# pain7576/ddpg-trucktrailer

Measured on AMD Instinct MI355X. Metric: env-steps/s, higher is better.
Workload: dtype f64

## Files before the change

### ddpg-trucktrailer_amd/_lib.py

```python
import ctypes as C
import os

HERE = os.path.dirname(os.path.abspath(__file__))
LIB_PATH = os.environ.get("TT_LIB_PATH") or os.path.join(HERE, "libttenv.so")

OBS_DIM = 23
MAX_EPISODE_STEPS = 4095
TT_OK, TT_EINVAL, TT_ENOMEM, TT_EHIP, TT_ENODEV = 0, -1, -2, -3, -4
F_JACKKNIFE, F_OUT_OF_MAP, F_MAX_STEPS, F_GOAL_REACHED, F_GOAL_PASSED, F_EXCESSIVE_BACK, F_SUCCESS = (1 << i for i in range(7))
VIOLATIONS = ("none", "jackknife", "jackknife_warning", "major_boundary", "minor_boundary", "past_the_goal",
              "max_step", "excessive_backward")
INFO_ROWS = ("total_reward", "progress_reward", "heading_reward", "orientation_reward", "staged_success",
             "safety_penalty", "exploration_bonus", "final_success_bonus", "backward_penalty", "smoothness_penalty",
             "cumulative_backward", "movement_budget")
NINFO = len(INFO_ROWS)
LOG_COUNTS = ("episodes", "successes", "jackknife", "out_of_map", "max_steps", "goal_reached", "goal_passed",
              "excessive_back", "success_flag")
LOG_DETAIL = 1
LOG_COMPONENTS = INFO_ROWS[1:10]


class TTParams(C.Structure):
    _fields_ = [(n, C.c_double) for n in ("L1", "L2", "hitch_offset", "v1x", "dt", "map_min_x", "map_max_x", "map_min_y",
                                          "map_max_y", "max_steer", "position_threshold", "orientation_threshold",
                                          "step_length")] + \
               [("extra_steps", C.c_int32), ("fixed_max_steps", C.c_int32), ("term_mask", C.c_uint32),
                ("variant", C.c_int32), ("stateless_reward", C.c_int32), ("reserved_", C.c_int32),
                ("goal", C.c_double * 3), ("reset_lo", C.c_double * 3),
                ("reset_hi", C.c_double * 3)]


class TTInfo(C.Structure):
    _fields_ = [("comp", C.c_void_p), ("violation", C.c_void_p), ("flags", C.c_void_p)]


class TTMlpWeights(C.Structure):
    _fields_ = [(n, C.c_void_p) for n in ("w1", "b1", "g1", "be1", "w2", "b2", "g2", "be2", "w3", "b3", "wa", "ba")] + \
               [("in_dim", C.c_int32), ("fc1_dims", C.c_int32), ("fc2_dims", C.c_int32), ("capped_grids", C.c_int32),
                ("split_ws", C.c_void_p), ("ws_packed", C.c_int32), ("max_workgroups", C.c_int32), ("split_ws_alt", C.c_void_p), ("fc2_img", C.c_void_p)]


class TTFc2Images(C.Structure):
    _fields_ = [("net", C.c_void_p), ("target", C.c_void_p)]


class TTMlpSaved(C.Structure):
    _fields_ = [(n, C.c_void_p) for n in ("xh1", "h1", "xh2", "h2", "rstd1", "rstd2")]


class TTFwdJob(C.Structure):
    _fields_ = [("critic", C.c_int32), ("reserved_", C.c_int32), ("obs", C.c_void_p), ("action", C.c_void_p),
                ("w", C.POINTER(TTMlpWeights)), ("out", C.c_void_p), ("saved", C.POINTER(TTMlpSaved)),
                ("dq_da", C.c_void_p), ("z_state", C.c_void_p)]


class TTTdInput(C.Structure):
    _fields_ = [("z_state", C.c_void_p), ("mu_target", C.c_void_p), ("target_critic", C.POINTER(TTMlpWeights)),
                ("reward", C.c_void_p), ("done", C.c_void_p), ("gamma", C.c_float), ("reserved_", C.c_float),
                ("y_out", C.c_void_p), ("q_out", C.c_void_p), ("step_dev", C.c_void_p), ("window_dev", C.c_void_p),
                ("bias_corr_out", C.c_void_p), ("adam_beta1", C.c_float), ("adam_beta2", C.c_float)]


class TTSideBuffer(C.Structure):
    _fields_ = [("obs", C.c_void_p), ("act", C.c_void_p), ("rew", C.c_void_p), ("obs2", C.c_void_p), ("done", C.c_void_p),
                ("count", C.c_int32), ("reserved_", C.c_int32)]


class TTRingView(C.Structure):
    _fields_ = [("cursor", C.c_void_p), ("obs", C.c_void_p), ("act", C.c_void_p), ("rew", C.c_void_p), ("done", C.c_void_p),
                ("n_envs", C.c_int32), ("slots", C.c_int32)]


class TTRingCursor(C.Structure):
    _fields_ = [("k_dev", C.c_void_p), ("slots", C.c_int32), ("reserved_", C.c_int32), ("cursor", C.c_void_p)]


class TTSampleArgs(C.Structure):
    _fields_ = [("batch", C.c_int32), ("n_envs", C.c_int32), ("slots", C.c_int32), ("reserve", C.c_int32), ("k_dev", C.c_void_p),
                ("obs", C.c_void_p), ("act", C.c_void_p), ("rew", C.c_void_p), ("done", C.c_void_p), ("seed", C.c_uint64),
                ("side", C.POINTER(TTSideBuffer)), ("s_out", C.c_void_p), ("a_out", C.c_void_p), ("r_out", C.c_void_p),
                ("s2_out", C.c_void_p), ("d_out", C.c_void_p), ("idx_out", C.c_void_p), ("lag", C.c_int32),
                ("draws", C.c_int32), ("seed_stride", C.c_uint64), ("step_progress", C.c_void_p)]


class TTImageJob(C.Structure):
    _fields_ = [("actor", C.POINTER(TTMlpWeights)), ("cursor", C.POINTER(TTRingCursor))]


class TTMlpBwdWs(C.Structure):
    _fields_ = [(n, C.c_void_p) for n in ("dpre", "dz", "dx2", "dy1", "dx1")]


class TTPopNet(C.Structure):
    _fields_ = [("ws", C.POINTER(TTMlpBwdWs)), ("grads", C.POINTER(TTMlpWeights)), ("count", C.c_int32), ("reserved_", C.c_int32),
                ("params", C.c_void_p), ("exp_avg", C.c_void_p), ("exp_avg_sq", C.c_void_p), ("targets", C.c_void_p)] + \
               [(n, C.c_float) for n in ("lr", "beta1", "beta2", "eps", "weight_decay", "tau")] + [("images", C.POINTER(TTFc2Images))]


class TTPopAgent(C.Structure):
    _fields_ = [("sample", C.POINTER(TTSampleArgs)), ("jobs", C.POINTER(TTFwdJob)), ("td", C.POINTER(TTTdInput)),
                ("critic", TTPopNet), ("actor", TTPopNet), ("q_pi", C.c_void_p), ("dq_da", C.c_void_p), ("tail_words", C.c_void_p),
                ("gave_up_host", C.c_void_p)]


class TTPopExploitPair(C.Structure):
    _fields_ = [("dst", C.c_int32), ("src", C.c_int32), ("alpha", C.c_float), ("beta", C.c_float), ("tau", C.c_float),
                ("gamma", C.c_float)]


class TTPopNstep(C.Structure):
    _fields_ = [("n_step", C.c_int32), ("gamma", C.c_float), ("discount", C.c_float)]


class TTTd3Agent(C.Structure):
    _fields_ = [("sample", C.POINTER(TTSampleArgs)), ("jobs", C.POINTER(TTFwdJob)), ("td", C.POINTER(TTTdInput)),
                ("critic", TTPopNet), ("critic_2", TTPopNet), ("actor", TTPopNet), ("z_state_2", C.c_void_p),
                ("target_critic_2", C.POINTER(TTMlpWeights)), ("target_noise", C.c_float), ("noise_clip", C.c_float),
                ("noise_seed", C.c_uint64), ("eps_out", C.c_void_p), ("y2_out", C.c_void_p), ("q2t_out", C.c_void_p),
                ("step_snapshot", C.c_void_p), ("actor_step_dev", C.c_void_p), ("actor_bias_corr_out", C.c_void_p),
                ("q_pi", C.c_void_p), ("dq_da", C.c_void_p), ("tail_words", C.c_void_p), ("gave_up_host", C.c_void_p)]


class TTPopTd3Pair(C.Structure):
    _fields_ = [("dst", C.c_int32), ("src", C.c_int32)] + \
               [(n, C.c_float) for n in ("alpha", "beta", "tau", "gamma", "target_noise", "noise_clip")]


class TTLearnLogJob(C.Structure):
    _fields_ = [(n, C.c_void_p) for n in ("y", "q", "q_pi", "dq_da", "mu", "grad_critic", "grad_actor")] + \
               [("numel_critic", C.c_int32), ("numel_actor", C.c_int32), ("step_dev", C.c_void_p)]


LEARN_LOG_VALUES = ("critic_loss", "actor_loss", "q_mean", "q_min", "q_max", "y_mean", "y_min", "y_max", "td_abs_mean", "td_abs_max",
                    "dq_da_abs_mean", "dq_da_abs_max", "mu_abs_mean", "gate_mean", "grad_norm_critic", "grad_norm_actor")
LEARN_LOG_CHUNKS = 16
LEARN_LOG_MAX_CAPACITY = 1 << 22
POP_MAX_AGENTS = 16
NSTEP_MAX = 16
TD3_NOISE_TAG = 0x7D3E


class TTError(RuntimeError):
    pass


_P, _I, _U64 = C.c_void_p, C.c_int, C.c_uint64
_SIGNATURES = {
    "tt_version": (C.c_int, []),
    "tt_last_error": (C.c_char_p, [_P]),
    "tt_params_default": (C.c_int, [_I, C.POINTER(TTParams)]),
    "tt_env_create": (C.c_int, [_I, _I, C.POINTER(TTParams), C.POINTER(_P)]),
    "tt_env_destroy": (C.c_int, [_P]),
    "tt_env_num_envs": (C.c_int, [_P]),
    "tt_env_reset": (C.c_int, [_P, _P, _U64, _P, _P]),
    "tt_env_set_reset_pool": (C.c_int, [_P, _P, _I]),
    "tt_env_set_pose": (C.c_int, [_P, _P, _I, _P, _P, _P, _P, _P]),
    "tt_env_set_attrs": (C.c_int, [_P, _P, _I, _P, _P, _P, _P]),
    "tt_env_set_state": (C.c_int, [_P, _P, _I, _P, _P]),
    "tt_env_get_state": (C.c_int, [_P, _P, _P]),
    "tt_env_set_max_steps": (C.c_int, [_P, _P, _I, _P, _P]),
    "tt_env_set_steps": (C.c_int, [_P, _P, _I, _P, _P]),
    "tt_env_get_episode": (C.c_int, [_P, _P, _P, _P, _P, _P, _P]),
    "tt_env_observe": (C.c_int, [_P, _P, _P, _P]),
    "tt_env_set_step_counter": (C.c_int, [_P, _P]),
    "tt_env_step": (C.c_int, [_P, _P, _P, _P, _P, C.POINTER(TTInfo), _I, _P]),
    "tt_env_step_random": (C.c_int, [_P, _U64, _P, _P, _P, _P, C.POINTER(TTInfo), _I, _P]),
    "tt_env_state_bytes": (C.c_size_t, [_P]),
    "tt_env_export": (C.c_int, [_P, _P, C.POINTER(C.c_uint64 * 4), _P]),
    "tt_env_import": (C.c_int, [_P, _P, C.POINTER(C.c_uint64 * 4), _P]),
    "tt_env_set_episode_log": (C.c_int, [_P, C.c_int64, _P]),
    "tt_env_drain_episode_log": (C.c_int, [_P, _P, _P, _P, _P, _P, _P, _P, _P, _P]),
    "tt_env_episode_log_bytes": (C.c_size_t, [_P]),
    "tt_env_export_episode_log": (C.c_int, [_P, _P, C.POINTER(C.c_uint64 * 2), _P]),
    "tt_env_import_episode_log": (C.c_int, [_P, _P, C.POINTER(C.c_uint64 * 2), _P]),
    "tt_env_set_episode_log2": (C.c_int, [_P, C.c_int64, C.c_uint32, _P]),
    "tt_env_drain_episode_log2": (C.c_int, [_P, _P, _P, _P, _P, _P, _P, _P, _P, _P, _P, _P]),
    "tt_env_rollout_random": (C.c_int, [_P, _I, _U64, _P, _P, _P, _P]),
    "tt_env_profile": (C.c_int, [_P, _I]),
    "tt_env_profile_read": (C.c_int, [_P, C.POINTER(C.c_double), C.POINTER(C.c_int64)]),
    "tt_mlp_split_ws_bytes": (C.c_uint64, []),
    "tt_mlp_split_pack": (C.c_int, [C.POINTER(TTMlpWeights), _I, _P, _P, C.POINTER(TTRingCursor), _P]),
    "tt_mlp_split_pack_and_sample": (C.c_int, [C.POINTER(TTMlpWeights), _I, _P, C.POINTER(TTSampleArgs), C.POINTER(TTRingCursor), _P]),
    "tt_actor_act_ring": (C.c_int, [_I, C.POINTER(TTRingView), C.POINTER(TTMlpWeights), _P, _U64, _U64, _P, C.c_float, C.c_float,
                                    C.c_float, _P, _P]),
    "tt_env_step_ring": (C.c_int, [_P, _P, C.POINTER(TTRingView), _I, _P]),
    "tt_actor_forward": (C.c_int, [_I, _P, C.POINTER(TTMlpWeights), _P, _P]),
    "tt_actor_act": (C.c_int, [_I, _P, C.POINTER(TTMlpWeights), _P, _P, _U64, _U64, _P, C.c_float, C.c_float, C.c_float,
                               _P, _P, _P, _P]),
    "tt_ring_sample": (C.c_int, [_I, _I, _I, _P, _P, _P, _P, _P, _U64, _I, _I, C.POINTER(TTSideBuffer), _P, _P, _P, _P, _P, _P, _P]),
    "tt_critic_forward": (C.c_int, [_I, _P, _P, C.POINTER(TTMlpWeights), _P, _P]),
    "tt_mlp_forward_save": (C.c_int, [_I, _I, _P, _P, C.POINTER(TTMlpWeights), _P, C.POINTER(TTMlpSaved), _P, _P]),
    "tt_mlp_forward_multi": (C.c_int, [_I, _I, C.POINTER(TTFwdJob), _P]),
    "tt_mlp_forward_multi_sampled": (C.c_int, [_I, _I, C.POINTER(TTFwdJob), C.POINTER(TTSampleArgs), _P, _P]),
    "tt_ring_sample_nstep": (C.c_int, [C.POINTER(TTSampleArgs), _I, C.c_float, _P]),
    "tt_mlp_forward_multi_sampled_nstep": (C.c_int, [_I, _I, C.POINTER(TTFwdJob), C.POINTER(TTSampleArgs), _I, C.c_float, _P, _P]),
    "tt_mlp_backward_rows_pair": (C.c_int, [_I, C.c_float, _P, C.POINTER(TTMlpWeights), C.POINTER(TTMlpSaved), C.POINTER(TTMlpBwdWs),
                                            C.POINTER(TTTdInput), _P, C.POINTER(TTMlpWeights), C.POINTER(TTMlpSaved),
                                            C.POINTER(TTMlpBwdWs), C.POINTER(TTImageJob), _P]),
    "tt_mlp_backward_weights": (C.c_int, [_I, _I, _P, _P, C.POINTER(TTMlpSaved), C.POINTER(TTMlpBwdWs), C.POINTER(TTMlpWeights),
                                          _P, _P, C.c_float, _I, _P, _P, _P, _P, _P, C.c_float, C.c_float, C.c_float, C.c_float,
                                          C.c_float, C.c_float, C.POINTER(TTFc2Images), _P, _P]),
    "tt_mlp_actor_tail": (C.c_int, [_I, _P, _P, C.POINTER(TTMlpWeights), _P, _P, C.POINTER(TTMlpSaved), C.POINTER(TTMlpBwdWs),
                                    C.POINTER(TTMlpWeights), C.c_float, _I, _P, _P, _P, _P, _P, C.c_float, C.c_float, C.c_float, C.c_float,
                                    C.c_float, C.c_float, C.POINTER(TTFc2Images), _P, _P, _P, _P]),
    "tt_adam_soft_update": (C.c_int, [_I, _P, _P, _P, _P, _P, _P, _P, C.c_float, C.c_float, C.c_float, C.c_float,
                                      C.c_float, C.c_float, C.POINTER(TTFc2Images), _P, _P]),
    "tt_p2p_create": (C.c_int, [_I, _I, _I, _I, _P, C.POINTER(_P)]),
    "tt_p2p_destroy": (C.c_int, [_P]),
    "tt_p2p_export": (C.c_int, [_P, _P]),
    "tt_p2p_attach": (C.c_int, [_P, _I, _P]),
    "tt_p2p_grad": (_P, [_P, _I]),
    "tt_p2p_reset": (C.c_int, [_P, _P]),
    "tt_p2p_set_timeout": (C.c_int, [_P, C.c_double]),
    "tt_p2p_gave_up": (C.c_int, [_P]),
    "tt_p2p_last_error": (C.c_char_p, [_P]),
    "tt_adam_soft_update_p2p": (C.c_int, [_P, _I, _I, _P, _P, _P, _P, _P, _P, C.c_float, C.c_float, C.c_float, C.c_float,
                                          C.c_float, C.c_float, C.POINTER(TTFc2Images), _P, _P]),
    "tt_mlp_fc2_image_bytes": (C.c_uint64, []),
    "tt_mlp_fc2_image_pack": (C.c_int, [C.POINTER(TTMlpWeights), _P]),
    "tt_random_actions": (C.c_int, [_I, _U64, _U64, _P, _P]),
    "tt_pop_learn_create": (C.c_int, [_I, _I, C.POINTER(TTPopAgent), C.POINTER(_P)]),
    "tt_pop_learn": (C.c_int, [_P, _I, _P]),
    "tt_pop_learn_destroy": (C.c_int, [_P]),
    "tt_pop_exploit": (C.c_int, [_P, _I, C.POINTER(TTPopExploitPair), _P]),
    "tt_pop_hyper": (C.c_int, [_P, _I, C.POINTER(C.c_float * 4)]),
    "tt_pop_learn_set_nstep": (C.c_int, [_P, C.POINTER(TTPopNstep)]),
    "tt_pop_exploit_nstep": (C.c_int, [_P, _I, C.POINTER(TTPopExploitPair), C.POINTER(TTPopNstep), _P]),
    "tt_pop_nstep": (C.c_int, [_P, _I, C.POINTER(TTPopNstep)]),
    "tt_learn_log_create": (C.c_int, [_I, _I, C.POINTER(TTLearnLogJob), C.c_int64, C.c_int32, C.POINTER(_P)]),
    "tt_learn_log_append": (C.c_int, [_P, _P]),
    "tt_learn_log_drain": (C.c_int, [_P, _I, C.c_int64, C.c_int64, _P, _P, _P, C.POINTER(C.c_int64)]),
    "tt_learn_log_clear": (C.c_int, [_P, _P]),
    "tt_learn_log_destroy": (C.c_int, [_P]),
    "tt_td3_create": (C.c_int, [_I, C.POINTER(TTTd3Agent), C.POINTER(_P)]),
    "tt_td3_update": (C.c_int, [_P, C.POINTER(TTTd3Agent)]),
    "tt_td3_learn": (C.c_int, [_P, _I, _I, _P]),
    "tt_td3_destroy": (C.c_int, [_P]),
    "tt_pop_td3_create": (C.c_int, [_I, _I, C.POINTER(TTTd3Agent), C.POINTER(_P)]),
    "tt_pop_td3_learn": (C.c_int, [_P, _I, _I, _P]),
    "tt_pop_td3_exploit": (C.c_int, [_P, _I, C.POINTER(TTPopTd3Pair), _P]),
    "tt_pop_td3_hyper": (C.c_int, [_P, _I, C.POINTER(C.c_float * 6)]),
    "tt_pop_td3_destroy": (C.c_int, [_P]),
}
EXPORTS = tuple(_SIGNATURES)

_lib = None


def load():
    global _lib
    if _lib is None:
        if not os.path.exists(LIB_PATH):
            raise ImportError(f"{LIB_PATH} is missing: build it with `python -c 'import __graft_entry__ as g; g.build()'` "
                              "(hipcc --offload-arch=gfx950); there is no CPU fallback")
        import torch
        lib = C.CDLL(LIB_PATH)
        for name, (res, args) in _SIGNATURES.items():
            fn = getattr(lib, name)
            fn.restype, fn.argtypes = res, args
        _lib = lib
    return _lib


def ptr(t):
    return None if t is None else C.c_void_p(t.data_ptr())


def stream(device=None):
    import torch
    return C.c_void_p(torch.cuda.current_stream(device).cuda_stream)


def check(rc, handle=None):
    if rc != TT_OK:
        msg = load().tt_last_error(handle)
        raise TTError(f"libttenv error {rc}: {msg.decode() if msg else '?'}")


def check_p2p(rc, handle=None):
    if rc != TT_OK:
        msg = load().tt_p2p_last_error(handle)
        raise TTError(f"libttenv p2p error {rc}: {msg.decode() if msg else '?'}")


P2P_HANDLE_BYTES, P2P_MAX_RANKS = 128, 8


def default_params(variant=0):
    p = TTParams()
    check(load().tt_params_default(variant, C.byref(p)))
    return p
```

### ddpg-trucktrailer_amd/build.py

```python
import os
import shutil
import subprocess

HERE = os.path.dirname(os.path.abspath(__file__))
ROOT = os.path.dirname(HERE)
SRC = [os.path.join(HERE, "csrc", f) for f in ("ttenv.hip", "ttnet.hip", "ttnet_split.hip", "ttlearn.hip", "ttp2p.hip", "ttpop.hip", "ttnstep.hip", "ttpop_nstep.hip", "ttlearnlog.hip", "tttd3.hip", "ttpop_td3.hip")]
HDR = [os.path.join(ROOT, "include", "ttenv.h"), os.path.join(HERE, "csrc", "ttnet_common.h"), os.path.join(HERE, "csrc", "ttnet_pack.h"), os.path.join(HERE, "csrc", "ttp2p.h"), os.path.join(HERE, "csrc", "ttstamps.h"), os.path.join(HERE, "csrc", "ttlearn_bodies.h"), os.path.join(HERE, "csrc", "ttnstep.h"), os.path.join(HERE, "csrc", "ttpop.h"), os.path.join(HERE, "csrc", "tthost.h"), os.path.join(HERE, "csrc", "ttphilox.h"), os.path.join(HERE, "csrc", "tttd3.h")]
LIB = os.path.join(HERE, "libttenv.so")


def hipcc():
    for c in (os.environ.get("HIPCC"), shutil.which("hipcc"), "/opt/rocm/bin/hipcc"):
        if c and os.path.exists(c):
            return c
    raise RuntimeError("hipcc not found (set HIPCC)")


def stale():
    if not os.path.exists(LIB):
        return True
    t = os.path.getmtime(LIB)
    return any(os.path.getmtime(p) > t for p in SRC + HDR)


def build(force=False, verbose=False, defines=(), out=None):
    if out is None and not force and not stale():
        return LIB
    out = out or LIB
    cmd = [hipcc(), "--offload-arch=gfx950", "-O3", "-std=c++17", "-fPIC", "-shared", "-mllvm", "-amdgpu-kernarg-preload-count=16",
           "-I" + os.path.join(ROOT, "include"), "-o", out] + ["-D" + d for d in defines] + SRC
    if verbose:
        print(" ".join(cmd))
    subprocess.check_call(cmd)
    return out


VARIANTS = {
    "stamps": (("TT_STAMPS",), os.path.join(ROOT, "tools", "dbg", "libttenv_stamps.so")),
}


def build_variant(name, verbose=False):
    defines, out = VARIANTS[name]
    os.makedirs(os.path.dirname(out), exist_ok=True)
    if os.path.exists(out) and all(os.path.getmtime(p) <= os.path.getmtime(out) for p in SRC + HDR):
        return out
    return build(force=True, verbose=verbose, defines=defines, out=out)


if __name__ == "__main__":
    import sys
    if len(sys.argv) > 2 and sys.argv[1] == "--variant":
        print(build_variant(sys.argv[2], verbose=True))
    else:
        print(build(force=True, verbose=True))
```

### ddpg-trucktrailer_amd/csrc/ttnet.hip

```cpp
#include <cstdio>
#include <cstdlib>

#include "ttnet_common.h"

using namespace ttnet;

namespace {

constexpr int INP = 24;
constexpr int H2P = 320;
constexpr int NT1 = H1 / 16;
constexpr int NT2 = H2P / 16;
constexpr int BM = 64, WROWS = 16;

using f32x4 = __attribute__((ext_vector_type(4))) float;

template <int CTRL>
__device__ __forceinline__ float dpp_f(float v) {
    return __builtin_bit_cast(float, __builtin_amdgcn_update_dpp(0, __builtin_bit_cast(int, v), CTRL, 0xf, 0xf, true));
}
__device__ __forceinline__ float row_sum16(float v) {
    v += dpp_f<0xB1>(v);
    v += dpp_f<0x4E>(v);
    v += dpp_f<0x141>(v);
    v += dpp_f<0x140>(v);
    return v;
}

constexpr int HS2 = 404;
constexpr int V2_LDS_BYTES = (BM * HS2 + H1 * IN + 3 * H1 + 6 * H2) * 4;

template <bool CRITIC>
__global__ __launch_bounds__(256, 1) void k_mlp_forward_v2(const int n, const float *__restrict__ obs,
                                                           const float *__restrict__ action, const Weights W,
                                                           float *__restrict__ out, const ActArgs act) {
    extern __shared__ __attribute__((aligned(16))) float lds[];
    float *h1_s = lds;
    float *w1_s = h1_s + BM * HS2;
    float *p1_s = w1_s + H1 * IN;
    float *p2_s = p1_s + 3 * H1;
    const int tid = threadIdx.x, wave = tid >> 6, lane = tid & 63;
    const int l15 = lane & 15, l4 = lane >> 4;
    const int row0 = blockIdx.x * BM, wrow0 = row0 + wave * WROWS;

    {
        const float4 *src = reinterpret_cast<const float4 *>(W.w1);
        float4 *dst = reinterpret_cast<float4 *>(w1_s);
        for (int i = tid; i < H1 * IN / 4; i += 256) dst[i] = src[i];
        for (int i = tid; i < H1; i += 256) { p1_s[i] = W.b1[i]; p1_s[H1 + i] = W.g1[i]; p1_s[2 * H1 + i] = W.be1[i]; }
        for (int i = tid; i < H2; i += 256) {
            p2_s[i] = W.b2[i]; p2_s[H2 + i] = W.g2[i]; p2_s[2 * H2 + i] = W.be2[i]; p2_s[3 * H2 + i] = W.w3[i];
            if (CRITIC) { p2_s[4 * H2 + i] = W.wa[i]; p2_s[5 * H2 + i] = W.ba[i]; }
        }
    }
    f32x4 acc1[NT1];
#pragma unroll
    for (int t = 0; t < NT1; ++t) acc1[t] = f32x4{0.f, 0.f, 0.f, 0.f};
    {
        float a[INP / 4];
#pragma unroll
        for (int ks = 0; ks < INP / 4; ++ks) {
            const int k = ks * 4 + l4;
            a[ks] = (k < IN && wrow0 + l15 < n) ? resolve_obs(act, obs)[(size_t)(wrow0 + l15) * IN + k] : 0.f;
        }
        __syncthreads();
#pragma unroll
        for (int t = 0; t < NT1; ++t) {
            float b[INP / 4];
#pragma unroll
            for (int ks = 0; ks < INP / 4; ++ks) {
                const int k = ks * 4 + l4;
                b[ks] = k < IN ? w1_s[(t * 16 + l15) * IN + k] : 0.f;
            }
#pragma unroll
            for (int ks = 0; ks < INP / 4; ++ks) acc1[t] = __builtin_amdgcn_mfma_f32_16x16x4f32(a[ks], b[ks], acc1[t], 0, 0, 0);
        }
    }
    {
        float s[4] = {0.f, 0.f, 0.f, 0.f};
#pragma unroll
        for (int t = 0; t < NT1; ++t) {
            const float bias = p1_s[t * 16 + l15];
#pragma unroll
            for (int r = 0; r < 4; ++r) { acc1[t][r] += bias; s[r] += acc1[t][r]; }
        }
        float mean[4], rstd[4], ss[4] = {0.f, 0.f, 0.f, 0.f};
#pragma unroll
        for (int r = 0; r < 4; ++r) mean[r] = row_sum16(s[r]) * (1.f / H1);
#pragma unroll
        for (int t = 0; t < NT1; ++t)
#pragma unroll
            for (int r = 0; r < 4; ++r) { const float d = acc1[t][r] - mean[r]; ss[r] = fmaf(d, d, ss[r]); }
#pragma unroll
        for (int r = 0; r < 4; ++r) rstd[r] = rsqrtf(row_sum16(ss[r]) * (1.f / H1) + 1e-5f);
#pragma unroll
        for (int t = 0; t < NT1; ++t) {
            const int col = t * 16 + l15;
            const float g = p1_s[H1 + col], be = p1_s[2 * H1 + col];
#pragma unroll
            for (int r = 0; r < 4; ++r)
                h1_s[(wave * WROWS + l4 * 4 + r) * HS2 + col] = fmaxf(fmaf((acc1[t][r] - mean[r]) * rstd[r], g, be), 0.f);
        }
    }
    __builtin_amdgcn_s_waitcnt(0xc07f);
    __builtin_amdgcn_wave_barrier();

    f32x4 acc2[NT2];
#pragma unroll
    for (int t = 0; t < NT2; ++t) acc2[t] = f32x4{0.f, 0.f, 0.f, 0.f};
    constexpr int SS = 2, NSS = (H1 / 16 + SS - 1) / SS;
    struct BFrag { float4 v[SS][NT2]; };
    const float *wbase = W.w2 + (size_t)l15 * H1 + 4 * l4;
    auto load_b = [&](int ss) {
        BFrag f;
#pragma unroll
        for (int st = 0; st < SS; ++st) {
            const int c = ss * SS + st;
#pragma unroll
            for (int t = 0; t < NT2; ++t) {
                const bool real = c < H1 / 16 && t * 16 + l15 < H2;
                f.v[st][t] = real ? *reinterpret_cast<const float4 *>(wbase + (size_t)t * 16 * H1 + 16 * c)
                                  : make_float4(0.f, 0.f, 0.f, 0.f);
            }
        }
        return f;
    };
    const float *arow = h1_s + (wave * WROWS + l15) * HS2 + 4 * l4;
    BFrag cur = load_b(0);
    for (int ss = 0; ss < NSS; ++ss) {
        BFrag nxt = cur;
        if (ss + 1 < NSS) nxt = load_b(ss + 1);
#pragma unroll
        for (int st = 0; st < SS; ++st) {
            const int c = ss * SS + st;
            if (c < H1 / 16) {
                const float4 av = *reinterpret_cast<const float4 *>(arow + 16 * c);
#pragma unroll
                for (int t = 0; t < NT2; ++t) acc2[t] = __builtin_amdgcn_mfma_f32_16x16x4f32(av.x, cur.v[st][t].x, acc2[t], 0, 0, 0);
#pragma unroll
                for (int t = 0; t < NT2; ++t) acc2[t] = __builtin_amdgcn_mfma_f32_16x16x4f32(av.y, cur.v[st][t].y, acc2[t], 0, 0, 0);
#pragma unroll
                for (int t = 0; t < NT2; ++t) acc2[t] = __builtin_amdgcn_mfma_f32_16x16x4f32(av.z, cur.v[st][t].z, acc2[t], 0, 0, 0);
#pragma unroll
                for (int t = 0; t < NT2; ++t) acc2[t] = __builtin_amdgcn_mfma_f32_16x16x4f32(av.w, cur.v[st][t].w, acc2[t], 0, 0, 0);
            }
        }
        cur = nxt;
    }

    float s[4] = {0.f, 0.f, 0.f, 0.f};
#pragma unroll
    for (int t = 0; t < NT2; ++t) {
        const int col = t * 16 + l15;
        const bool real = col < H2;
        const float bias = real ? p2_s[col] : 0.f;
#pragma unroll
        for (int r = 0; r < 4; ++r) { acc2[t][r] = real ? acc2[t][r] + bias : 0.f; s[r] += acc2[t][r]; }
    }
    float mean[4], rstd[4];
#pragma unroll
    for (int r = 0; r < 4; ++r) mean[r] = row_sum16(s[r]) * (1.f / H2);
    float ss2[4] = {0.f, 0.f, 0.f, 0.f};
#pragma unroll
    for (int t = 0; t < NT2; ++t) {
        const bool real = t * 16 + l15 < H2;
#pragma unroll
        for (int r = 0; r < 4; ++r) { const float d = real ? acc2[t][r] - mean[r] : 0.f; ss2[r] = fmaf(d, d, ss2[r]); }
    }
#pragma unroll
    for (int r = 0; r < 4; ++r) rstd[r] = rsqrtf(row_sum16(ss2[r]) * (1.f / H2) + 1e-5f);
    float av[4] = {0.f, 0.f, 0.f, 0.f};
    if (CRITIC) {
#pragma unroll
        for (int r = 0; r < 4; ++r) {
            const int row = wrow0 + l4 * 4 + r;
            av[r] = row < n ? action[row] : 0.f;
        }
    }
    float dot[4] = {0.f, 0.f, 0.f, 0.f};
#pragma unroll
    for (int t = 0; t < NT2; ++t) {
        const int col = t * 16 + l15;
        if (col < H2) {
            const float g = p2_s[H2 + col], be = p2_s[2 * H2 + col], w3 = p2_s[3 * H2 + col];
            float wa = 0.f, ba = 0.f;
            if (CRITIC) { wa = p2_s[4 * H2 + col]; ba = p2_s[5 * H2 + col]; }
#pragma unroll
            for (int r = 0; r < 4; ++r) {
                float y = fmaf((acc2[t][r] - mean[r]) * rstd[r], g, be);
                if (CRITIC) y += fmaf(av[r], wa, ba);
                dot[r] = fmaf(fmaxf(y, 0.f), w3, dot[r]);
            }
        }
    }
    const float b3 = W.b3[0];
#pragma unroll
    for (int r = 0; r < 4; ++r) {
        const float v = row_sum16(dot[r]) + b3;
        const int row = wrow0 + l4 * 4 + r;
        if (l15 == 0 && row < n) finish_row<CRITIC>(row, v, out, act);
    }
}

int check_ptrs(const tt_mlp_weights *w, bool critic) {
    if (!w) return 0;
    if (w->in_dim != IN || w->fc1_dims != H1 || w->fc2_dims != H2) return 0;
    if (!w->w1 || !w->b1 || !w->g1 || !w->be1 || !w->w2 || !w->b2 || !w->g2 || !w->be2 || !w->w3 || !w->b3) return 0;
    if (critic && (!w->wa || !w->ba)) return 0;
    return 1;
}


bool use_split(int n, const tt_mlp_weights *w) {
    static int forced = -1;
    if (forced < 0) {
        const char *e = getenv("TT_MLP_KERNEL");
        forced = !e ? 0 : (e[0] == 'f' ? 1 : (e[0] == 's' ? 2 : 0));
    }
    if (!w->split_ws) return false;
    if (w->ws_packed) return true;
    if (forced == 1) return false;
    return forced == 2 || n >= 1024;
}

template <bool CRITIC>
int launch(int n, const float *obs, const float *action, const tt_mlp_weights *w, float *out, const ActArgs &act,
           hipStream_t stream) {
    if (use_split(n, w)) {
        const int rc = w->ws_packed ? TT_OK : split_pack(w, CRITIC, w->split_ws, nullptr, RingCursor{nullptr, 0, nullptr}, stream);
        return rc != TT_OK ? rc : split_forward(CRITIC, n, obs, action, w, out, act, stream);
    }
    static bool attr2[64] = {};
    int dev = 0;
    if (hipGetDevice(&dev) != hipSuccess || dev < 0 || dev >= 64) return TT_EHIP;
    if (!attr2[dev]) {
        if (hipFuncSetAttribute(reinterpret_cast<const void *>(&k_mlp_forward_v2<CRITIC>),
                                hipFuncAttributeMaxDynamicSharedMemorySize, V2_LDS_BYTES) != hipSuccess)
            return TT_EHIP;
        attr2[dev] = true;
    }
    hipLaunchKernelGGL((k_mlp_forward_v2<CRITIC>), dim3((n + BM - 1) / BM), dim3(256), V2_LDS_BYTES, stream, n, obs,
                       action, to_weights(w), out, act);
    return hipGetLastError() == hipSuccess ? TT_OK : TT_EHIP;
}

__global__ __launch_bounds__(64) void k_ring_sample(const RingSample R) {
    if ((int)blockIdx.x < R.batch) ring_sample_row(R, blockIdx.x, threadIdx.x);
}

}

extern "C" {

#ifdef TT_STAMPS
int tt_debug_nstamps(unsigned long long *out16) { return ttnet::split_debug_stamps(out16); }
int tt_debug_bstamps(unsigned long long *out, int nblocks) { return ttnet::split_debug_block_stamps(out, nblocks); }
int tt_debug_policy_tiles(unsigned long long *out4096) { return ttnet::split_debug_tiles(out4096); }
int tt_debug_policy_poll(unsigned long long *out4) { return ttnet::split_debug_poll(out4); }
int tt_debug_log_policy(unsigned long long *out, int reset) { return ttnet::split_debug_log(out, reset); }
#endif

uint64_t tt_mlp_split_ws_bytes(void) { return (uint64_t)split_ws_bytes(); }

static RingCursor to_cursor(const tt_ring_cursor *c) {
    return (c && c->cursor && c->k_dev && c->slots > 0)
               ? RingCursor{reinterpret_cast<const long long *>(c->k_dev), c->slots, c->cursor} : RingCursor{nullptr, 0, nullptr};
}

int tt_mlp_split_pack(const tt_mlp_weights *w, int critic, void *ws, int64_t *bump, const tt_ring_cursor *cursor,
                      tt_stream_t stream) {
    if (!ws || !check_ptrs(w, critic != 0)) return TT_EINVAL;
    if (bump && cursor && bump == cursor->k_dev) return TT_EINVAL;
    return split_pack(w, critic != 0, ws, reinterpret_cast<long long *>(bump), to_cursor(cursor), stream);
}

int tt_actor_forward(int n, const float *obs, const tt_mlp_weights *w, float *mu_out, tt_stream_t stream) {
    if (n < 0 || !obs || !mu_out || !check_ptrs(w, false)) return TT_EINVAL;
    if (n == 0) return TT_OK;
    ActArgs act{};
    return launch<false>(n, obs, nullptr, w, mu_out, act, stream);
}

static ActArgs act_args(float *ou_state, const uint8_t *done_prev, float *act_raw, float *act_scaled, const int64_t *step_dev,
                        uint64_t seed, uint64_t step, float theta_dt, float sigma_sqrt_dt, float high) {
    ActArgs act{};
    act.ou = ou_state; act.done_prev = done_prev; act.act_raw = act_raw; act.act_scaled = act_scaled;
    act.step_dev = reinterpret_cast<const long long *>(step_dev);
    act.seed = seed; act.step = step;
    act.decay = 1.0f - theta_dt; act.scale = sigma_sqrt_dt; act.high = high;
    return act;
}

int tt_actor_act(int n, const float *obs, const tt_mlp_weights *w, float *ou_state, const uint8_t *done_prev,
                 uint64_t seed, uint64_t step, const int64_t *step_dev, float theta_dt, float sigma_sqrt_dt, float high,
                 float *mu_out, float *act_raw_out, float *act_scaled_out, tt_stream_t stream) {
    if (n < 0 || !obs || !ou_state || !act_raw_out || !act_scaled_out || !check_ptrs(w, false)) return TT_EINVAL;
    if (n == 0) return TT_OK;
    const ActArgs act = act_args(ou_state, done_prev, act_raw_out, act_scaled_out, step_dev, seed, step, theta_dt, sigma_sqrt_dt, high);
    return launch<false>(n, obs, nullptr, w, mu_out, act, stream);
}

int tt_actor_act_ring(int n, const tt_ring_view *ring, const tt_mlp_weights *w, float *ou_state, uint64_t seed, uint64_t step,
                      const int64_t *step_dev, float theta_dt, float sigma_sqrt_dt, float high, float *act_scaled_out,
                      tt_stream_t stream) {
    if (n <= 0 || !ring || !ring->cursor || !ring->obs || !ring->act || !ring->done || ring->n_envs != n || !ou_state ||
        !step_dev || !act_scaled_out || !check_ptrs(w, false) || !w->split_ws || !w->ws_packed)
        return TT_EINVAL;
    ActArgs act = act_args(ou_state, ring->done, ring->act, act_scaled_out, step_dev, seed, step, theta_dt, sigma_sqrt_dt, high);
    act.cursor = ring->cursor; act.ring_n = n; act.ring_slots = ring->slots;
    return launch<false>(n, ring->obs, nullptr, w, nullptr, act, stream);
}

int tt_ring_sample(int batch, int n_envs, int slots, const int64_t *k_dev, const float *obs, const float *act,
                   const float *rew, const uint8_t *done, uint64_t seed, int reserve, int lag, const tt_side_buffer *side,
                   float *s_out, float *a_out, float *r_out, float *s2_out, uint8_t *d_out, int32_t *idx_out,
                   tt_stream_t stream) {
    const tt_sample_args a{batch, n_envs, slots, reserve, k_dev, obs, act, rew, done, seed, side, s_out, a_out, r_out, s2_out,
                           d_out, idx_out, lag, 1, 0, nullptr};
    RingSample R;
    const int rc = make_ring_sample(&a, R);
    if (rc != TT_OK || batch == 0) return rc;
    hipLaunchKernelGGL(k_ring_sample, dim3(batch), dim3(64), 0, stream, R);
    return hipGetLastError() == hipSuccess ? TT_OK : TT_EHIP;
}

int tt_mlp_split_pack_and_sample(const tt_mlp_weights *w, int critic, void *ws, const tt_sample_args *a,
                                 const tt_ring_cursor *cursor, tt_stream_t stream) {
    if (!ws || !a || !check_ptrs(w, critic != 0)) return TT_EINVAL;
    RingSample R;
    const int rc = make_ring_sample(a, R);
    if (rc != TT_OK) return rc;
    if (a->draws < 0 || (long long)(a->draws > 1 ? a->draws : 1) * a->batch > (1 << 24)) return TT_EINVAL;
    if (a->draws > 1) { R.draws = a->draws; R.seed_stride = a->seed_stride; }
    return split_pack_and_sample(w, critic != 0, ws, R, to_cursor(cursor), stream);
}

int tt_critic_forward(int n, const float *obs, const float *action, const tt_mlp_weights *w, float *q_out,
                      tt_stream_t stream) {
    if (n < 0 || !obs || !action || !q_out || !check_ptrs(w, true)) return TT_EINVAL;
    if (n == 0) return TT_OK;
    ActArgs act{};
    return launch<true>(n, obs, action, w, q_out, act, stream);
}

}
```

### ddpg-trucktrailer_amd/csrc/ttnet_common.h

```cpp
#pragma once
#include <hip/hip_runtime.h>

#include <cstdint>

#include "ttenv.h"
#include "ttphilox.h"

namespace ttnet {

constexpr int IN = 23;
constexpr int H1 = 400, H2 = 300;

struct Weights {
    const float *w1, *b1, *g1, *be1;
    const float *w2, *b2, *g2, *be2;
    const float *w3, *b3;
    const float *wa, *ba;
};

struct ActArgs {
    float *ou;
    const uint8_t *done_prev;
    float *act_raw, *act_scaled;
    const long long *step_dev;
    unsigned long long seed, step;
    float decay, scale, high;
    int *cursor;
    int ring_n;
    int ring_slots;
};

__device__ __forceinline__ const int *cursor_of(const ActArgs &act) {
    return act.cursor + 4 + 4 * (int)(*act.step_dev & 1);
}
__device__ __forceinline__ const float *resolve_obs(const ActArgs &act, const float *obs) {
    return act.cursor ? obs + (size_t)cursor_of(act)[0] * act.ring_n * IN : obs;
}

using ttrng::philox4x32;

template <bool CRITIC>
__device__ __forceinline__ void finish_row(const int row, const float v, float *__restrict__ out, const ActArgs &act) {
    if (CRITIC) {
        out[row] = v;
        return;
    }
    const float mu = tanhf(v);
    if (out) out[row] = mu;
    if (act.ou) {
        float x = act.ou[row];
        const uint8_t *done_prev = act.done_prev;
        float *act_raw = act.act_raw;
        if (act.cursor) {
            const int *c = cursor_of(act);
            done_prev = c[3] ? act.done_prev + (size_t)c[2] * act.ring_n : nullptr;
            act_raw += (size_t)c[0] * act.ring_n;
        }
        if (done_prev && done_prev[row]) x = 0.f;
        const unsigned long long st = act.step + (act.step_dev ? (unsigned long long)*act.step_dev : 0ull);
        uint32_t rnd[4];
        philox4x32((uint32_t)row, (uint32_t)st, (uint32_t)(st >> 32), 0x0A5Eu, (uint32_t)act.seed,
                   (uint32_t)(act.seed >> 32), rnd);
        const float u1 = ((float)(rnd[0] >> 8) + 0.5f) * (1.f / 16777216.f);
        const float u2 = ((float)(rnd[1] >> 8) + 0.5f) * (1.f / 16777216.f);
        const float nrm = sqrtf(-2.f * logf(u1)) * cosf(6.28318530717958647692f * u2);
        x = fmaf(x, act.decay, act.scale * nrm);
        act.ou[row] = x;
        const float a = mu + x;
        act_raw[row] = a;
        act.act_scaled[row] = fminf(fmaxf(a, -1.f), 1.f) * act.high;
    }
}

__device__ __forceinline__ float ou_advance(const int row, const float x_prev, const bool restart, const ActArgs &act,
                                            const unsigned long long st) {
    float x = restart ? 0.f : x_prev;
    uint32_t rnd[4];
    philox4x32((uint32_t)row, (uint32_t)st, (uint32_t)(st >> 32), 0x0A5Eu, (uint32_t)act.seed, (uint32_t)(act.seed >> 32), rnd);
    const float u1 = ((float)(rnd[0] >> 8) + 0.5f) * (1.f / 16777216.f);
    const float u2 = ((float)(rnd[1] >> 8) + 0.5f) * (1.f / 16777216.f);
    const float nrm = sqrtf(-2.f * logf(u1)) * cosf(6.28318530717958647692f * u2);
    return fmaf(x, act.decay, act.scale * nrm);
}
__device__ __forceinline__ void finish_row_noise(const int row, const float v, float *__restrict__ out, const ActArgs &act,
                                                 const float x_new, float *__restrict__ act_raw) {
    const float mu = tanhf(v);
    if (out) out[row] = mu;
    act.ou[row] = x_new;
    const float a = mu + x_new;
    act_raw[row] = a;
    act.act_scaled[row] = fminf(fmaxf(a, -1.f), 1.f) * act.high;
}


struct SideBuf {
    const float *obs, *act, *rew, *obs2;
    const uint8_t *done;
    int count;
};
struct RingSample {
    int batch, n_envs, slots, reserve, lag;
    const long long *k_dev;
    const float *obs, *act, *rew;
    const uint8_t *done;
    unsigned long long seed;
    SideBuf side;
    float *s_out, *a_out, *r_out, *s2_out;
    uint8_t *d_out;
    int *idx_out;
    int draws;
    unsigned long long seed_stride;
    int *progress;
};

struct RingPick {
    bool side;
    int j, t, t1, e;
};
__device__ inline RingPick ring_sample_index(const RingSample &R, const int b, const unsigned long long seed) {
    const int n_envs = R.n_envs, slots = R.slots;
    const long long k0 = *R.k_dev - R.lag, k = k0 > 0 ? k0 : 0;
    const long long cap = slots - 1 - R.reserve;
    const long long avail = k < cap ? k : cap;
    uint32_t r[4];
    philox4x32((uint32_t)b, (uint32_t)k, (uint32_t)(k >> 32), 0x5A3Du, (uint32_t)seed, (uint32_t)(seed >> 32), r);
    RingPick p{false, 0, 0, 0, 0};
    if (R.side.count > 0) {
        const unsigned long long in_ring = (unsigned long long)avail * (unsigned long long)n_envs;
        const unsigned long long u = ((unsigned long long)r[2] << 32) | r[3];
        if (__umul64hi(u, in_ring + (unsigned long long)R.side.count) < (unsigned long long)R.side.count) {
            p.side = true;
            p.j = (int)(((unsigned long long)r[0] * (unsigned long long)R.side.count) >> 32);
            return p;
        }
    }
    const long long back = avail > 0 ? (long long)(((unsigned long long)r[0] * (unsigned long long)avail) >> 32) : 0;
    p.t = (int)(((k - 1 - back) % slots + slots) % slots);
    p.t1 = (p.t + 1) % slots;
    p.e = (int)(((unsigned long long)r[1] * (unsigned long long)n_envs) >> 32);
    return p;
}
__device__ inline RingPick ring_sample_index(const RingSample &R, const int b) { return ring_sample_index(R, b, R.seed); }
__device__ __forceinline__ const float *ring_pick_s(const RingSample &R, const RingPick &p) {
    return p.side ? R.side.obs + (size_t)p.j * IN : R.obs + ((size_t)p.t * R.n_envs + p.e) * IN;
}
__device__ __forceinline__ const float *ring_pick_s2(const RingSample &R, const RingPick &p) {
    return p.side ? R.side.obs2 + (size_t)p.j * IN : R.obs + ((size_t)p.t1 * R.n_envs + p.e) * IN;
}
__device__ __forceinline__ float ring_pick_a(const RingSample &R, const RingPick &p) {
    return p.side ? R.side.act[p.j] : R.act[(size_t)p.t * R.n_envs + p.e];
}
__device__ __forceinline__ float ring_pick_r(const RingSample &R, const RingPick &p) {
    return p.side ? R.side.rew[p.j] : R.rew[(size_t)p.t * R.n_envs + p.e];
}
__device__ __forceinline__ uint8_t ring_pick_d(const RingSample &R, const RingPick &p) {
    return p.side ? R.side.done[p.j] : R.done[(size_t)p.t * R.n_envs + p.e];
}

__device__ inline void ring_sample_row(const RingSample &R, const int b, const int lane) {
    const int u = R.draws > 1 ? b / R.batch : 0;
    const RingPick p = ring_sample_index(R, b - u * R.batch, R.seed + (unsigned long long)u * R.seed_stride);
    const float *src = ring_pick_s(R, p), *src2 = ring_pick_s2(R, p);
    if (lane < IN) R.s_out[(size_t)b * IN + lane] = src[lane];
    else if (lane >= 32 && lane < 32 + IN) R.s2_out[(size_t)b * IN + lane - 32] = src2[lane - 32];
    if (lane == 63) {
        R.a_out[b] = ring_pick_a(R, p);
        R.r_out[b] = ring_pick_r(R, p);
        R.d_out[b] = ring_pick_d(R, p);
        if (R.idx_out) { R.idx_out[2 * b] = p.side ? -1 : p.t; R.idx_out[2 * b + 1] = p.side ? p.j : p.e; }
    }
}

inline int make_ring_sample(const tt_sample_args *a, RingSample &R) {
    if (!a || a->batch < 0 || a->n_envs <= 0 || a->reserve < 0 || a->lag < 0 || a->slots < 3 + a->reserve || !a->k_dev || !a->obs ||
        !a->act || !a->rew || !a->done || !a->s_out || !a->a_out || !a->r_out || !a->s2_out || !a->d_out)
        return TT_EINVAL;
    SideBuf sb{nullptr, nullptr, nullptr, nullptr, nullptr, 0};
    if (a->side && a->side->count > 0) {
        const tt_side_buffer *sd = a->side;
        if (!sd->obs || !sd->act || !sd->rew || !sd->obs2 || !sd->done) return TT_EINVAL;
        sb = SideBuf{sd->obs, sd->act, sd->rew, sd->obs2, sd->done, sd->count};
    }
    R = RingSample{a->batch, a->n_envs, a->slots, a->reserve, a->lag, reinterpret_cast<const long long *>(a->k_dev), a->obs, a->act,
                   a->rew, a->done, a->seed, sb, a->s_out, a->a_out, a->r_out, a->s2_out, a->d_out, a->idx_out, 1, 0ull, nullptr};
    return TT_OK;
}

inline Weights to_weights(const tt_mlp_weights *w) {
    return Weights{w->w1, w->b1, w->g1, w->be1, w->w2, w->b2, w->g2, w->be2, w->w3, w->b3, w->wa, w->ba};
}

struct RingCursor {
    const long long *k_dev;
    int slots;
    int *cursor;
};
__device__ __forceinline__ void write_cursor(const RingCursor &c) {
    if (!c.cursor) return;
    const long long k = *c.k_dev;
    int *out = c.cursor + 4 + 4 * (int)(k & 1);
    out[0] = (int)(k % c.slots);
    out[1] = (int)((k + 1) % c.slots);
    out[2] = (int)((k + c.slots - 1) % c.slots);
    out[3] = k > 0 ? 1 : 0;
}

#ifdef TT_STAMPS
static __device__ unsigned long long g_poll[4];
#define TT_POLL(i) atomicAdd(&g_poll[i], 1ull)
#else
#define TT_POLL(i) do { } while (0)
#endif
constexpr int CUR_EPOCH = 12, CUR_ARRIVED = 14, CUR_GAVE_UP = 15, CUR_PROGRESS = 16, CUR_GAVE_UP_MIRROR = 18;
constexpr unsigned long long TT_IMAGE_WAIT_TICKS = 25000000ull;
__device__ __forceinline__ void mark_gave_up(int *cursor, const int value) {
    __hip_atomic_store(cursor + CUR_GAVE_UP, value, __ATOMIC_RELAXED, __HIP_MEMORY_SCOPE_AGENT);
    int *mirror = *reinterpret_cast<int *const *>(cursor + CUR_GAVE_UP_MIRROR);
    if (mirror) __hip_atomic_store(mirror, value, __ATOMIC_RELAXED, __HIP_MEMORY_SCOPE_SYSTEM);
}
__device__ __forceinline__ void publish_image(const RingCursor &c, const int workgroups) {
    asm volatile("s_waitcnt vmcnt(0)" ::: "memory");
    __syncthreads();
    if (threadIdx.x == 0 && c.cursor) {
        __builtin_amdgcn_fence(__ATOMIC_RELEASE, "agent");
        asm volatile("s_waitcnt vmcnt(0)" ::: "memory");
        const int before = __hip_atomic_fetch_add(c.cursor + CUR_ARRIVED, 1, __ATOMIC_RELAXED, __HIP_MEMORY_SCOPE_AGENT);
        if (before == workgroups - 1) {
            const long long k = *c.k_dev;
            __hip_atomic_store(c.cursor + CUR_ARRIVED, 0, __ATOMIC_RELAXED, __HIP_MEMORY_SCOPE_AGENT);
            __hip_atomic_store(c.cursor + CUR_EPOCH + (int)(k & 1), (int)(k + 1), __ATOMIC_RELAXED, __HIP_MEMORY_SCOPE_AGENT);
        }
    }
}
struct EpochPair { int e[2]; };
__device__ __forceinline__ EpochPair await_image_early(int *cursor) {
    EpochPair p{{0, 0}};
    if (cursor && threadIdx.x == 0) {
        p.e[0] = __hip_atomic_load(cursor + CUR_EPOCH, __ATOMIC_RELAXED, __HIP_MEMORY_SCOPE_AGENT);
        p.e[1] = __hip_atomic_load(cursor + CUR_EPOCH + 1, __ATOMIC_RELAXED, __HIP_MEMORY_SCOPE_AGENT);
    }
    return p;
}
__device__ __forceinline__ void await_image(int *cursor, const long long *step_dev, const EpochPair early = EpochPair{{0, 0}}) {
    if (!cursor) return;
    if (threadIdx.x == 0) {
        const long long k = *step_dev;
        const int want = (int)(k + 1);
        const int *flag = cursor + CUR_EPOCH + (int)(k & 1);
        if (early.e[k & 1] - want >= 0 || __hip_atomic_load(flag, __ATOMIC_RELAXED, __HIP_MEMORY_SCOPE_AGENT) - want >= 0) TT_POLL(0);
        else {
            TT_POLL(1);
            const unsigned long long t0 = wall_clock64();
            while (__hip_atomic_load(flag, __ATOMIC_RELAXED, __HIP_MEMORY_SCOPE_AGENT) - want < 0) {
                __builtin_amdgcn_s_sleep(127);
                if (wall_clock64() - t0 > TT_IMAGE_WAIT_TICKS) {
                    mark_gave_up(cursor, want);
                    break;
                }
            }
            __builtin_amdgcn_fence(__ATOMIC_ACQUIRE, "agent");
            asm volatile("s_waitcnt vmcnt(0)" ::: "memory");
        }
    }
    asm volatile("" ::: "memory");
    __syncthreads();
}

__device__ __forceinline__ void await_progress(int *progress, const long long *k_dev) {
    if (!progress) return;
    if (threadIdx.x == 0) {
        const int want = (int)*k_dev;
        if (__hip_atomic_load(progress, __ATOMIC_RELAXED, __HIP_MEMORY_SCOPE_AGENT) - want >= 0) TT_POLL(2);
        else {
            TT_POLL(3);
            const unsigned long long t0 = wall_clock64();
            while (__hip_atomic_load(progress, __ATOMIC_RELAXED, __HIP_MEMORY_SCOPE_AGENT) - want < 0) {
                __builtin_amdgcn_s_sleep(32);
                if (wall_clock64() - t0 > TT_IMAGE_WAIT_TICKS) {
                    mark_gave_up(progress - CUR_PROGRESS, want + 1);
                    break;
                }
            }
            __builtin_amdgcn_fence(__ATOMIC_ACQUIRE, "agent");
            asm volatile("s_waitcnt vmcnt(0)" ::: "memory");
        }
    }
    asm volatile("" ::: "memory");
    __syncthreads();
}

size_t split_ws_bytes();
int split_pack(const tt_mlp_weights *w, bool critic, void *ws, long long *bump, const RingCursor &cur, hipStream_t stream);
int split_pack_and_sample(const tt_mlp_weights *w, bool critic, void *ws, const RingSample &R, const RingCursor &cur,
                          hipStream_t stream);
int split_forward(bool critic, int n, const float *obs, const float *action, const tt_mlp_weights *w, float *out,
                  const ActArgs &act, hipStream_t stream);
#ifdef TT_STAMPS
int split_debug_stamps(unsigned long long *out16);
int split_debug_tiles(unsigned long long *out4096);
int split_debug_poll(unsigned long long *out4);
int split_debug_log(unsigned long long *out, int reset);
int split_debug_block_stamps(unsigned long long *out, int nblocks);
#endif

}
```

### ddpg-trucktrailer_amd/csrc/ttnet_split.hip

```cpp
#include "ttnet_common.h"
#include "ttnet_pack.h"
#include "ttstamps.h"

namespace ttnet {
namespace {

#ifdef TT_STAMPS
__device__ unsigned long long g_nstamps[16];
__device__ unsigned long long g_bstamps[4096 * 8];
#define NSTAMP(i) do { if (threadIdx.x == 0) { const unsigned long long w_ = wall_clock64();                                \
        if (blockIdx.x < 4096) { g_bstamps[blockIdx.x * 8 + (i)] = w_;                                                      \
            if ((i) == 0) g_bstamps[blockIdx.x * 8 + 7] = __builtin_amdgcn_s_getreg((20 << 0) | (0 << 6) | (3 << 11)); }     \
        if (blockIdx.x == 0) { g_nstamps[i] = w_; g_nstamps[8 + i] = clock64(); } } } while (0)
__device__ unsigned long long g_tile[512][4][2];
__device__ TTLog g_log_tile;
#define TSTAMP(round, e) do { if (threadIdx.x == 0 && blockIdx.x < 512 && (round) < 4) g_tile[blockIdx.x][round][e] = wall_clock64(); } while (0)
#else
#define NSTAMP(i) do { } while (0)
#define TSTAMP(round, e) do { } while (0)
#endif

__global__ __launch_bounds__(256) void k_split_pack(const Weights W, const bool critic, unsigned char *__restrict__ ws,
                                                    unsigned char *__restrict__ ws_alt, long long *__restrict__ bump,
                                                    const RingCursor cur) {
    split_pack_body(W, critic, ws, ws_alt, bump, cur, blockIdx.x * 256 + threadIdx.x);
    publish_image(cur, PACK_BLOCKS);
}

__global__ __launch_bounds__(256) void k_pack_and_sample(const Weights W, const bool critic, unsigned char *__restrict__ ws,
                                                         unsigned char *__restrict__ ws_alt, const RingSample R,
                                                         const RingCursor cur) {
    if ((int)blockIdx.x < PACK_BLOCKS) {
        split_pack_body(W, critic, ws, ws_alt, nullptr, cur, blockIdx.x * 256 + threadIdx.x);
        publish_image(cur, PACK_BLOCKS);
        return;
    }
    const int b = ((int)blockIdx.x - PACK_BLOCKS) * 4 + (threadIdx.x >> 6);
    if (b < R.batch * R.draws) ring_sample_row(R, b, threadIdx.x & 63);
}

constexpr int JOB_NONE = -1, JOB_FC1 = 100, JOB_NEXT = 200;
constexpr int TAIL0 = STEPS - (RING - 1);
constexpr int l2_job(const int s, const int u) {
    if (s == 0) return AHEAD - 1 + u / 5;
    if (s == 1 && u < 5) return RING - 1;
    if (u < 5) return JOB_NONE;
    if (s < TAIL0) return s + RING - 1;
    const int i = 5 * (s - TAIL0) + u - 5;
    if (i < W1_WAVE_PIECES) return JOB_FC1 + i;
    if (s == TAIL0 + 3 || s == TAIL0 + 4) return JOB_NEXT + s - (TAIL0 + 3);
    return JOB_NONE;
}
constexpr int l2_piece(const int u) { return u % 5; }
constexpr int job_slot(const int j) { return j >= JOB_NEXT ? j - JOB_NEXT : (j >= JOB_FC1 ? W1_OFF / CHUNK_BYTES + (j - JOB_FC1) / 5 : j % RING); }
constexpr bool l2_slots_free() {
    for (int s = 0; s < STEPS; ++s)
        for (int u = 0; u < T2; ++u) {
            const int j = l2_job(s, u);
            if (j == JOB_NONE) continue;
            if (s == 0 || (s == 1 && u < 5)) { if (job_slot(j) < W1_OFF / CHUNK_BYTES) return false; }
            else if (u < 5 || job_slot(j) != (s - 1) % RING) return false;
        }
    return true;
}
static_assert(l2_slots_free(), "a piece of layer 2 overwrites a slot that may still be read");
constexpr int mid_allowed(const int s) {
    int n = 10, after = s + 1 == 2 ? 5 : (s + 1 == 3 ? 10 : -1000);
    for (int ss = 0; ss < STEPS; ++ss)
        for (int u = 0; u < T2; ++u) {
            if (ss == s && u == T2 / 2) return n - after;
            const int j = l2_job(ss, u);
            if (j != JOB_NONE) { ++n; if (j == s + 1) after = n; }
        }
    return -1;
}
constexpr bool mid_counts_ok() {
    for (int s = 1; s + 1 < STEPS; ++s) if (mid_allowed(s) != (s < TAIL0 + 3 ? 20 : 18)) return false;
    return true;
}
static_assert(mid_counts_ok(), "the counted waits of layer 2 do not match the issue schedule");
struct L2Schedule {
    int job[STEPS][T2], mid[STEPS];
};
constexpr L2Schedule make_l2_schedule() {
    L2Schedule t{};
    for (int s = 0; s < STEPS; ++s) {
        t.mid[s] = mid_allowed(s);
        for (int u = 0; u < T2; ++u) t.job[s][u] = l2_job(s, u);
    }
    return t;
}
constexpr L2Schedule L2S = make_l2_schedule();

using lds_b = const __attribute__((address_space(3))) unsigned char;
using v4u = __attribute__((ext_vector_type(4))) unsigned;
struct LdsBases {
    lds_b *b0, *b1, *b2;
};
__device__ __forceinline__ uint4 lds_frag(const LdsBases &L, const int off) {
    lds_b *p = (off >> 16) == 0 ? L.b0 : ((off >> 16) == 1 ? L.b1 : L.b2);
    const v4u t = *(const __attribute__((address_space(3))) v4u *)(p + (off & 0xFFFF));
    return make_uint4(t[0], t[1], t[2], t[3]);
}

template <bool CRITIC>
__global__ __launch_bounds__(256, 1) void k_mlp_split(const int n, const int tile0, const int tile_end,
                                                      int *__restrict__ cursor_e, const long long *__restrict__ step_e,
                                                      const float *__restrict__ obs,
                                                      const unsigned char *__restrict__ ws,
                                                      const unsigned char *__restrict__ ws_alt,
                                                      const float *__restrict__ action, float *__restrict__ out,
                                                      const ActArgs act) {
    extern __shared__ __attribute__((aligned(16))) unsigned char lds_raw[];
    const float *p1_s = reinterpret_cast<const float *>(lds_raw + RING_BYTES);
    const int tid = threadIdx.x, lane = tid & 63;
    const int wave = __builtin_amdgcn_readfirstlane(tid >> 6);
    const int r = lane & 31, h = lane >> 5;
    using lds_f = const __attribute__((address_space(3))) float;
    using v4 = __attribute__((ext_vector_type(4))) float;
    auto lds4 = [](lds_f *q) -> float4 {
        const v4 t = *(const __attribute__((address_space(3))) v4 *)q;
        return make_float4(t[0], t[1], t[2], t[3]);
    };
    lds_f *pv1_0 = (lds_f *)(p1_s + 4 * h);
    LdsBases LB0;
    LB0.b0 = (lds_b *)lds_raw + lane * 16;
    LB0.b1 = LB0.b0 + 65536;
    LB0.b2 = LB0.b0 + 131072;
    const EpochPair epochs = await_image_early(cursor_e);
    const long long kstep = cursor_e ? *step_e : 0;
    const bool odd = act.cursor && (kstep & 1);
    const bool local = act.cursor && act.ring_slots > 0;
    const int slot_t = !local ? 0 : ((unsigned long long)kstep >> 32) == 0ull ? (int)((unsigned)kstep % (unsigned)act.ring_slots)
                                                                             : (int)(kstep % act.ring_slots);
    const float *obs_base = local ? obs + (size_t)slot_t * act.ring_n * IN : obs;
    const unsigned lds_base0 = (unsigned)(uintptr_t)(__attribute__((address_space(3))) unsigned char *)lds_raw;
    auto dma_piece = [&](const unsigned char *base, const unsigned voff, const unsigned lds_wave, const unsigned dst_const)
                         __attribute__((always_inline)) {
        unsigned keep;
        asm volatile("s_mov_b32 %0, m0\n\ts_add_u32 m0, %3, %4\n\ts_nop 0\n\tglobal_load_lds_dwordx4 %1, %2\n\ts_mov_b32 m0, %0"
                     : "=&s"(keep) : "v"(voff), "s"(base), "s"(lds_wave), "s"(dst_const) : "memory", "scc");
    };
    const unsigned voff_w2 = lane * 16 + wave * 5120 + WS_W2;
    const unsigned voff_w1 = lane * 16 + wave * 1024 + WS_W1;
    const unsigned voff_vec = lane * 16 + wave * (VEC_PIECES / 4) * 1024 + WS_VEC;
    const unsigned ldsw_w2_0 = lds_base0 + wave * 5120, ldsw_w1_0 = lds_base0 + W1_OFF + wave * 1024;
    auto issue_fc1_piece = [&](const unsigned char *w, const unsigned ldsw_w1, const int i) __attribute__((always_inline)) {
        dma_piece(w, voff_w1 + i * 4096, ldsw_w1, i * 4096);
    };
    auto issue_step_piece = [&](const unsigned char *w, const unsigned ldsw_w2, const int s, const int i) __attribute__((always_inline)) {
        dma_piece(w, voff_w2 + s * CHUNK_BYTES + i * 1024, ldsw_w2, (s % RING) * CHUNK_BYTES + i * 1024);
    };
    float xo[S1][8];
    float ou_pre = 0.f;
    unsigned dp_pre = 0u;
    const bool with_noise = !CRITIC && act.ou != nullptr;
    const uint8_t *dprev = act.done_prev;
    float *araw = act.act_raw;
    auto load_obs = [&](const int tile) __attribute__((always_inline)) {
        const int row = tile * ROWS + wave * WROWS + r;
        const int rowc = row < n ? row : n - 1;
        const float *orow = obs_base + (size_t)rowc * IN;
#pragma unroll
        for (int s = 0; s < S1; ++s)
#pragma unroll
            for (int j = 0; j < 8; ++j) {
                const int k = 16 * s + 8 * h + j;
                xo[s][j] = orow[k < IN ? k : IN - 1];
            }
        if (with_noise) {
            ou_pre = act.ou[rowc];
            dp_pre = dprev ? (unsigned)dprev[rowc] : 0u;
        }
    };

    NSTAMP(0);
    int tile = tile0 + (int)blockIdx.x;
    if (tile >= tile_end) return;
    if (local) {
        const int sl = act.ring_slots;
        const int slot_prev = slot_t == 0 ? sl - 1 : slot_t - 1;
        dprev = kstep > 0 ? act.done_prev + (size_t)slot_prev * act.ring_n : nullptr;
        araw = act.act_raw + (size_t)slot_t * act.ring_n;
    }
    if (!act.cursor || local) load_obs(tile);
    await_image(act.cursor, act.step_dev, epochs);
    const unsigned char *wsl = (odd && ws_alt) ? ws_alt : ws;
    if (act.cursor && !local) {
        obs_base = resolve_obs(act, obs);
        const int *c = cursor_of(act);
        dprev = c[3] ? act.done_prev + (size_t)c[2] * act.ring_n : nullptr;
        araw = act.act_raw + (size_t)c[0] * act.ring_n;
        load_obs(tile);
    }
    const unsigned long long noise_step = act.step + (act.step_dev ? (unsigned long long)*act.step_dev : 0ull);
    if (act.cursor && tile0 == 0 && blockIdx.x == 0 && tid == 0)
        __hip_atomic_store(act.cursor + CUR_PROGRESS, (int)(kstep + 1), __ATOMIC_RELAXED, __HIP_MEMORY_SCOPE_AGENT);
    if (act.cursor && tile0 == 0 && blockIdx.x == 0 && tid < 4) {
        const int sl = act.ring_slots;
        act.cursor[tid] = !local ? cursor_of(act)[tid]
                                 : (tid == 0 ? slot_t : tid == 1 ? (slot_t + 1 == sl ? 0 : slot_t + 1)
                                                      : tid == 2 ? (slot_t == 0 ? sl - 1 : slot_t - 1) : (kstep > 0 ? 1 : 0));
    }
#pragma unroll
    for (int i = 0; i < W1_WAVE_PIECES; ++i) issue_fc1_piece(wsl, ldsw_w1_0, i);
#pragma unroll
    for (int i = 0; i < VEC_PIECES / 4; ++i)
        dma_piece(wsl, voff_vec + i * 1024, lds_base0 + RING_BYTES + wave * (VEC_PIECES / 4) * 1024, i * 1024);
    bool first = true;
#ifdef TT_STAMPS
    int round = 0;
    if (threadIdx.x == 0 && blockIdx.x < 512) for (int q = 0; q < 4; ++q) g_tile[blockIdx.x][q][0] = g_tile[blockIdx.x][q][1] = 0ull;
    if (threadIdx.x == 0 && blockIdx.x < 512) g_tile[blockIdx.x][0][0] = wall_clock64();
#endif

#pragma unroll 1
    for (;;) {
        const unsigned char *wsl_cur = wsl;
        unsigned ldsw_w2 = ldsw_w2_0, ldsw_w1 = ldsw_w1_0;
        LdsBases LB = LB0;
        lds_f *pv1 = pv1_0;
        asm volatile("" : "+s"(wsl_cur), "+s"(ldsw_w2), "+s"(ldsw_w1), "+v"(LB.b0), "+v"(LB.b1), "+v"(LB.b2), "+v"(pv1));
        lds_f *pv2 = pv1 + 2 * H1P;
        const int row = tile * ROWS + wave * WROWS + r;
#pragma unroll
        for (int s = 0; s < S1; ++s)
#pragma unroll
            for (int j = 0; j < 8; ++j) {
                const int k = 16 * s + 8 * h + j;
                xo[s][j] = k < IN ? (row < n ? xo[s][j] : 0.f) : (k == IN ? 1.f : 0.f);
            }
        float ou_next = 0.f;
        if (with_noise) ou_next = ou_advance(row < n ? row : n - 1, ou_pre, dp_pre != 0u, act, noise_step);
        uint4 xb[S1][2];
#pragma unroll
        for (int s = 0; s < S1; ++s) {
            uint32_t ph[4], pm[4];
#pragma unroll
            for (int p = 0; p < 4; ++p) split2(xo[s][2 * p] * SX, xo[s][2 * p + 1] * SX, ph[p], pm[p]);
            xb[s][0] = make_uint4(ph[0], ph[1], ph[2], ph[3]);
            xb[s][1] = make_uint4(pm[0], pm[1], pm[2], pm[3]);
        }
        asm volatile("s_waitcnt vmcnt(0)" ::: "memory");
        __builtin_amdgcn_s_barrier();
        if (first) NSTAMP(1);

#define SB __builtin_amdgcn_sched_barrier(0)
        f32x16 acc1[T1];
        {
            auto w1_frag = [&](const int q, const int plane) __attribute__((always_inline)) {
                return lds_frag(LB, W1_OFF + (((q % S1) * T1 + q / S1) * 2 + plane) * 1024);
            };
            const unsigned char *wsl_1 = wsl_cur;
            asm volatile("" : "+s"(wsl_1));
            uint4 a0h = w1_frag(0, 0), a0m = w1_frag(0, 1), a1h = w1_frag(1, 0), a1m = w1_frag(1, 1), a2h = a0h, a2m = a0m;
            SB;
#pragma unroll
            for (int q = 0; q < S1 * T1; ++q) {
                const int t = q / S1, s = q % S1;
                if (s == 0) {
#pragma unroll
                    for (int v = 0; v < 16; ++v) acc1[t][v] = 0.f;
                }
                acc1[t] = mfma_f16(a0m, xb[s][0], acc1[t]); SB;
                if (q + 2 < S1 * T1) a2h = w1_frag(q + 2, 0);
                SB;
                acc1[t] = mfma_f16(a0h, xb[s][1], acc1[t]); SB;
                if (q + 2 < S1 * T1) a2m = w1_frag(q + 2, 1);
                SB;
                acc1[t] = mfma_f16(a0h, xb[s][0], acc1[t]); SB;
                if (q < 10) { if (first) issue_step_piece(wsl_1, ldsw_w2, q / 5, q % 5); }
                else if (q < 20) issue_step_piece(wsl_1, ldsw_w2, 2 + (q - 10) / 5, q % 5);
                SB;
                a0h = a1h; a0m = a1m; a1h = a2h; a1m = a2m;
            }
        }
        if (first) NSTAMP(2);
        uint32_t hb[STEPS][4], mb[STEPS][4];
        f32x2 nmean, rstdp;
        {
            f32x2 sp = pk(0.f, 0.f);
#pragma unroll
            for (int t = 0; t < T1; ++t)
#pragma unroll
                for (int v = 0; v < (t == T1 - 1 ? 8 : 16); v += 4)
                    sp += pk(acc1[t][v], acc1[t][v + 1]) + pk(acc1[t][v + 2], acc1[t][v + 3]);
            const float s = sp[0] + sp[1];
            const float mean = (s + __shfl_xor(s, 32)) * (1.f / H1);
            nmean = pk(-mean, -mean);
            f32x2 ssp = pk(0.f, 0.f);
#pragma unroll
            for (int t = 0; t < T1; ++t)
#pragma unroll
                for (int v = 0; v < (t == T1 - 1 ? 8 : 16); v += 2) {
                    const f32x2 d = pk(acc1[t][v], acc1[t][v + 1]) + nmean;
                    ssp = pk_fma(d, d, ssp);
                }
            const float ss = ssp[0] + ssp[1];
            const float var = (ss + __shfl_xor(ss, 32)) * (1.f / H1) * (UNSCALE * UNSCALE);
            const float rstd = rsqrtf(var + 1e-5f) * UNSCALE;
            rstdp = pk(rstd, rstd);
        }
        constexpr int GROUPS = 2 * STEPS;
        float4 gq[2], bq[2];
        f32x2 ya, yb;
        float y0, y1, y2, y3;
        auto ln_read = [&](const int G) __attribute__((always_inline)) {
            gq[G & 1] = lds4(pv1 + 8 * G);
            bq[G & 1] = lds4(pv1 + H1P + 8 * G);
        };
        auto ln_chunk = [&](const int G, const int k) __attribute__((always_inline)) {
            const int t = G >> 2, i = G & 3, st = G >> 1, e = 2 * (G & 1);
            const float4 g = gq[G & 1], be = bq[G & 1];
            if (k == 0) ya = pk_fma((pk(acc1[t][4 * i], acc1[t][4 * i + 1]) + nmean) * rstdp, pk(g.x, g.y), pk(be.x, be.y));
            if (k == 1) yb = pk_fma((pk(acc1[t][4 * i + 2], acc1[t][4 * i + 3]) + nmean) * rstdp, pk(g.z, g.w), pk(be.z, be.w));
            if (k == 2) {
                y0 = fmaxf(ya[0], 0.f); y1 = fmaxf(ya[1], 0.f); y2 = fmaxf(yb[0], 0.f); y3 = fmaxf(yb[1], 0.f);
                if (G + 1 < GROUPS) ln_read(G + 1);
            }
            if (k == 3) split2(y0, y1, hb[st][e], mb[st][e]);
            if (k == 4) split2(y2, y3, hb[st][e + 1], mb[st][e + 1]);
        };
        ln_read(0);
#pragma unroll
        for (int G = 0; G < 4; ++G)
#pragma unroll
            for (int k = 0; k < 5; ++k) ln_chunk(G, k);

        if (first) NSTAMP(3);
        f32x16 acc2[T2];
#pragma unroll
        for (int u = 0; u < T2; ++u)
#pragma unroll
            for (int v = 0; v < 16; ++v) acc2[u][v] = 0.f;
        asm volatile("s_waitcnt vmcnt(10)" ::: "memory");
        __builtin_amdgcn_s_barrier();
        uint4 c0h = lds_frag(LB, 0), c0m = lds_frag(LB, 1024), c1h = lds_frag(LB, 2048), c1m = lds_frag(LB, 3072), c2h = c0h, c2m = c0m;
        SB;
        auto l2_step = [&](const int s) __attribute__((always_inline)) {
            const uint4 vh = make_uint4(hb[s][0], hb[s][1], hb[s][2], hb[s][3]), vm = make_uint4(mb[s][0], mb[s][1], mb[s][2], mb[s][3]);
            const int slot = (s % RING) * CHUNK_BYTES, nslot = ((s + 1) % RING) * CHUNK_BYTES;
            const unsigned char *wsl_s = wsl_cur;
            unsigned lds_s = ldsw_w2, lds1_s = ldsw_w1;
            asm volatile("" : "+s"(wsl_s), "+s"(lds_s));
            if (s >= TAIL0 && s < TAIL0 + 3) asm volatile("" : "+s"(lds1_s));
#pragma unroll
            for (int u = 0; u < T2; ++u) {
                if (u == T2 / 2 && s >= 1 && s + 1 < STEPS) {
                    switch (L2S.mid[s]) {
                        case 20: asm volatile("s_waitcnt vmcnt(20)" ::: "memory"); break;
                        default: asm volatile("s_waitcnt vmcnt(18)" ::: "memory"); break;
                    }
                    __builtin_amdgcn_s_barrier();
                    SB;
                }
                const bool more = u + 2 < T2 || s + 1 < STEPS;
                const int nx = u + 2 < T2 ? slot + (u + 2) * 2048 : nslot + (u + 2 - T2) * 2048;
                acc2[u] = mfma_f16(c0h, vm, acc2[u]); SB;
                if (more) c2h = lds_frag(LB, nx);
                if (s + 2 < STEPS) ln_chunk(2 * (s + 2) + u / 5, u % 5);
                SB;
                acc2[u] = mfma_f16(c0m, vh, acc2[u]); SB;
                if (more) c2m = lds_frag(LB, nx + 1024);
                SB;
                acc2[u] = mfma_f16(c0h, vh, acc2[u]); SB;
                {
                    const int j = L2S.job[s][u];
                    const bool f1 = j >= JOB_FC1 && j < JOB_NEXT;
                    const int st = j >= JOB_NEXT ? j - JOB_NEXT : j, i1 = j - JOB_FC1;
                    if (j != JOB_NONE)
                        dma_piece(wsl_s, f1 ? voff_w1 + i1 * 4096 : voff_w2 + st * CHUNK_BYTES + l2_piece(u) * 1024, f1 ? lds1_s : lds_s,
                                  f1 ? i1 * 4096 : (st % RING) * CHUNK_BYTES + l2_piece(u) * 1024);
                }
                SB;
                c0h = c1h; c0m = c1m; c1h = c2h; c1m = c2m;
            }
        };
#pragma unroll
        for (int s = 0; s < 2; ++s) l2_step(s);
#pragma unroll
        for (int s = 2; s < TAIL0; ++s) l2_step(s);
#pragma unroll
        for (int s = TAIL0; s < STEPS; ++s) l2_step(s);
#undef SB

        if (first) NSTAMP(4);
        const int next = tile + (int)gridDim.x;
        const bool more_tiles = next < tile_end;
        if (more_tiles) load_obs(next);
        f32x2 s2p = pk(0.f, 0.f);
        {
            float4 bq[2][4];
            auto ldb = [&](const int u, float4 (&b)[4]) {
#pragma unroll
                for (int i = 0; i < 4; ++i) b[i] = lds4(pv2 + 32 * u + 8 * i);
            };
            ldb(0, bq[0]);
#pragma unroll
            for (int u = 0; u < T2; ++u) {
                if (u + 1 < T2) ldb(u + 1, bq[(u + 1) & 1]);
                __builtin_amdgcn_sched_barrier(0);
#pragma unroll
                for (int i = 0; i < 4; ++i) {
                    const float4 b = bq[u & 1][i];
                    const f32x2 xa = pk_fma(pk(acc2[u][4 * i], acc2[u][4 * i + 1]), pk(UNSCALE, UNSCALE), pk(b.x, b.y));
                    const f32x2 xb2 = pk_fma(pk(acc2[u][4 * i + 2], acc2[u][4 * i + 3]), pk(UNSCALE, UNSCALE), pk(b.z, b.w));
                    acc2[u][4 * i] = xa[0]; acc2[u][4 * i + 1] = xa[1]; acc2[u][4 * i + 2] = xb2[0]; acc2[u][4 * i + 3] = xb2[1];
                    s2p += xa + xb2;
                }
                __builtin_amdgcn_sched_barrier(0);
            }
        }
        const float s2 = s2p[0] + s2p[1];
        const float mean2 = (s2 + __shfl_xor(s2, 32)) * (1.f / H2);
        const f32x2 nmean2 = pk(-mean2, -mean2);
        f32x2 ss2p = pk(0.f, 0.f);
#pragma unroll
        for (int u = 0; u < T2; ++u)
#pragma unroll
            for (int i = 0; i < 4; ++i) {
                const bool real = 32 * u + 8 * i + 4 * h < H2;
                const f32x2 keep = real ? pk(1.f, 1.f) : pk(0.f, 0.f);
#pragma unroll
                for (int j = 0; j < 4; j += 2) {
                    const f32x2 d = pk(acc2[u][4 * i + j], acc2[u][4 * i + j + 1]) + nmean2;
                    acc2[u][4 * i + j] = d[0]; acc2[u][4 * i + j + 1] = d[1];
                    const f32x2 dk = (32 * u + 8 * i + 4 < H2) ? d : d * keep;
                    ss2p = pk_fma(dk, dk, ss2p);
                }
            }
        const float ss2 = ss2p[0] + ss2p[1];
        const float rstd2 = rsqrtf((ss2 + __shfl_xor(ss2, 32)) * (1.f / H2) + 1e-5f);
        const f32x2 rstd2p = pk(rstd2, rstd2);
        const float av = (CRITIC && row < n) ? action[row] : 0.f;
        f32x2 dotp = pk(0.f, 0.f);
        {
            constexpr int NV = CRITIC ? 5 : 3;
            float4 vq[2][4][NV];
            auto ldv = [&](const int u, float4 (&v)[4][NV]) {
#pragma unroll
                for (int i = 0; i < 4; ++i)
#pragma unroll
                    for (int q = 0; q < NV; ++q) v[i][q] = lds4(pv2 + (q + 1) * H2P + 32 * u + 8 * i);
            };
            ldv(0, vq[0]);
#pragma unroll
            for (int u = 0; u < T2; ++u) {
                if (u + 1 < T2) ldv(u + 1, vq[(u + 1) & 1]);
                __builtin_amdgcn_sched_barrier(0);
#pragma unroll
                for (int i = 0; i < 4; ++i) {
                    const float4 g = vq[u & 1][i][0], be = vq[u & 1][i][1], w3 = vq[u & 1][i][2];
                    f32x2 ya = pk_fma(pk(acc2[u][4 * i], acc2[u][4 * i + 1]) * rstd2p, pk(g.x, g.y), pk(be.x, be.y));
                    f32x2 yb = pk_fma(pk(acc2[u][4 * i + 2], acc2[u][4 * i + 3]) * rstd2p, pk(g.z, g.w), pk(be.z, be.w));
                    if (CRITIC) {
                        const float4 wa = vq[u & 1][i][NV - 2], ba = vq[u & 1][i][NV - 1];
                        ya += pk_fma(pk(av, av), pk(wa.x, wa.y), pk(ba.x, ba.y));
                        yb += pk_fma(pk(av, av), pk(wa.z, wa.w), pk(ba.z, ba.w));
                    }
                    dotp = pk_fma(pk(fmaxf(ya[0], 0.f), fmaxf(ya[1], 0.f)), pk(w3.x, w3.y), dotp);
                    dotp = pk_fma(pk(fmaxf(yb[0], 0.f), fmaxf(yb[1], 0.f)), pk(w3.z, w3.w), dotp);
                }
                __builtin_amdgcn_sched_barrier(0);
            }
        }
        const float dot = dotp[0] + dotp[1];
        const float v = dot + __shfl_xor(dot, 32) + lds4(pv1 - 4 * h + VEC_FLOATS).x;
        if (h == 0 && row < n) {
            if (with_noise) finish_row_noise(row, v, out, act, ou_next, araw);
            else finish_row<CRITIC>(row, v, out, act);
        }
        if (first) NSTAMP(5);
#ifdef TT_STAMPS
        TSTAMP(round, 1);
        if (threadIdx.x == 0 && blockIdx.x < 512 && round < 4) tt_log_add(g_log_tile, g_tile[blockIdx.x][round][0], g_tile[blockIdx.x][round][1]);
        ++round;
        if (more_tiles) TSTAMP(round, 0);
#endif
        if (!more_tiles) break;
        tile = next;
        first = false;
    }
    asm volatile("s_waitcnt vmcnt(0)" ::: "memory");
}

}

#ifdef TT_STAMPS
int split_debug_stamps(unsigned long long *out16) {
    return hipMemcpyFromSymbol(out16, HIP_SYMBOL(g_nstamps), sizeof(unsigned long long) * 16) == hipSuccess ? 0 : -3;
}
int split_debug_tiles(unsigned long long *out4096) {
    return hipMemcpyFromSymbol(out4096, HIP_SYMBOL(g_tile), sizeof(unsigned long long) * 512 * 4 * 2) == hipSuccess ? 0 : -3;
}
int split_debug_log(unsigned long long *out, int reset) {
    if (out && hipMemcpyFromSymbol(out, HIP_SYMBOL(g_log_tile), sizeof(TTLog)) != hipSuccess) return -3;
    if (reset) { const unsigned long long z = 0; if (hipMemcpyToSymbol(HIP_SYMBOL(g_log_tile), &z, sizeof(z)) != hipSuccess) return -3; }
    return 0;
}
int split_debug_poll(unsigned long long *out4) {
    return hipMemcpyFromSymbol(out4, HIP_SYMBOL(g_poll), sizeof(unsigned long long) * 4) == hipSuccess ? 0 : -3;
}
int split_debug_block_stamps(unsigned long long *out, int nblocks) {
    return hipMemcpyFromSymbol(out, HIP_SYMBOL(g_bstamps), sizeof(unsigned long long) * 8 * (nblocks < 4096 ? nblocks : 4096)) == hipSuccess ? 0 : -3;
}
#endif

size_t split_ws_bytes() { return (size_t)WS_BYTES; }

int split_pack(const tt_mlp_weights *w, bool critic, void *ws, long long *bump, const RingCursor &cur, hipStream_t stream) {
    unsigned char *alt = ws == w->split_ws ? reinterpret_cast<unsigned char *>(w->split_ws_alt) : nullptr;
    hipLaunchKernelGGL(k_split_pack, dim3(PACK_BLOCKS), dim3(256), 0, stream, to_weights(w), critic,
                       reinterpret_cast<unsigned char *>(ws), alt, bump, cur);
    return hipGetLastError() == hipSuccess ? TT_OK : TT_EHIP;
}

int split_pack_and_sample(const tt_mlp_weights *w, bool critic, void *ws, const RingSample &R, const RingCursor &cur,
                          hipStream_t stream) {
    unsigned char *alt = ws == w->split_ws ? reinterpret_cast<unsigned char *>(w->split_ws_alt) : nullptr;
    hipLaunchKernelGGL(k_pack_and_sample, dim3(PACK_BLOCKS + (R.batch * R.draws + 3) / 4), dim3(256), 0, stream, to_weights(w), critic,
                       reinterpret_cast<unsigned char *>(ws), alt, R, cur);
    return hipGetLastError() == hipSuccess ? TT_OK : TT_EHIP;
}

template <bool CRITIC>
static int launch_split(int n, const float *obs, const float *action, const tt_mlp_weights *w, float *out,
                        const ActArgs &act, hipStream_t stream) {
    static bool attr[64] = {};
    static int cus[64] = {};
    int dev = 0;
    if (hipGetDevice(&dev) != hipSuccess || dev < 0 || dev >= 64) return TT_EHIP;
    if (!attr[dev]) {
        if (hipFuncSetAttribute(reinterpret_cast<const void *>(&k_mlp_split<CRITIC>),
                                hipFuncAttributeMaxDynamicSharedMemorySize, LDS_BYTES) != hipSuccess)
            return TT_EHIP;
        int c = 0;
        if (hipDeviceGetAttribute(&c, hipDeviceAttributeMultiprocessorCount, dev) != hipSuccess || c <= 0) c = 256;
        cus[dev] = c;
        attr[dev] = true;
    }
    const int ntiles = (n + ROWS - 1) / ROWS;
    const int chip = cus[dev];
    int capped = 0;
    if (w->max_workgroups > 0) {
        const int limit = w->max_workgroups;
        capped = ntiles;
        if (w->capped_grids > 0 && (long long)w->capped_grids * limit < ntiles) capped = w->capped_grids * limit;
        const int rounds = (capped + limit - 1) / limit, g = (capped + rounds - 1) / rounds;
        hipLaunchKernelGGL((k_mlp_split<CRITIC>), dim3(g), dim3(256), LDS_BYTES, stream, n, 0, capped, act.cursor, act.step_dev, obs,
                           reinterpret_cast<const unsigned char *>(w->split_ws),
                           reinterpret_cast<const unsigned char *>(w->split_ws_alt), action, out, act);
    }
    if (capped < ntiles) {
        const int rest = ntiles - capped, rounds = (rest + chip - 1) / chip, g = (rest + rounds - 1) / rounds;
        hipLaunchKernelGGL((k_mlp_split<CRITIC>), dim3(g), dim3(256), LDS_BYTES, stream, n, capped, ntiles, act.cursor, act.step_dev, obs,
                           reinterpret_cast<const unsigned char *>(w->split_ws),
                           reinterpret_cast<const unsigned char *>(w->split_ws_alt), action, out, act);
    }
    return hipGetLastError() == hipSuccess ? TT_OK : TT_EHIP;
}

int split_forward(bool critic, int n, const float *obs, const float *action, const tt_mlp_weights *w, float *out,
                  const ActArgs &act, hipStream_t stream) {
    return critic ? launch_split<true>(n, obs, action, w, out, act, stream)
                  : launch_split<false>(n, obs, action, w, out, act, stream);
}

}
```

### ddpg-trucktrailer_amd/fused.py

```python
import contextlib
import ctypes as C
import math

import torch

from ddpg_trucktrailer_amd import _lib as L


def supported(net):
    if not all(hasattr(net, a) for a in ("fc1", "fc2", "bn1", "bn2")) or not (hasattr(net, "mu") or hasattr(net, "q")):
        return False
    return (net.fc1.weight.is_cuda and net.fc1.weight.dtype == torch.float32 and tuple(net.fc1.weight.shape) == (400, 23)
            and tuple(net.fc2.weight.shape) == (300, 400) and net.bn1.eps == 1e-5 and net.bn2.eps == 1e-5)


def pack_and_sample(net, index, sample_args, cursor=None):
    w = packed_weights_of(net, index)
    dev = net.fc2.weight.device
    L.check(L.load().tt_mlp_split_pack_and_sample(C.byref(w), 1 if hasattr(net, "action_value") else 0, C.c_void_p(w.split_ws),
                                                  C.byref(sample_args), C.byref(cursor) if cursor is not None else None,
                                                  L.stream(dev)))


def actor_act_ring(net, ring_view, weights, ou_state, act_scaled, seed, step=0, step_dev=None, theta=0.2, sigma=0.15, dt=1e-2,
                   high=math.pi / 4):
    dev = net.fc2.weight.device
    L.check(L.load().tt_actor_act_ring(int(ring_view.n_envs), C.byref(ring_view), C.byref(weights), L.ptr(ou_state),
                                       int(seed) & (2 ** 64 - 1), int(step), L.ptr(step_dev), float(theta * dt),
                                       float(sigma * math.sqrt(dt)), float(high), L.ptr(act_scaled),
                                       L.stream(dev)))
    return act_scaled


def _fill_weights(net, w):
    head = net.mu if hasattr(net, "mu") else net.q
    for name, t in (("w1", net.fc1.weight), ("b1", net.fc1.bias), ("g1", net.bn1.weight), ("be1", net.bn1.bias),
                    ("w2", net.fc2.weight), ("b2", net.fc2.bias), ("g2", net.bn2.weight), ("be2", net.bn2.bias),
                    ("w3", head.weight), ("b3", head.bias)):
        assert t.is_contiguous()
        setattr(w, name, t.data_ptr())
    if hasattr(net, "action_value"):
        w.wa, w.ba = net.action_value.weight.data_ptr(), net.action_value.bias.data_ptr()
    w.in_dim, w.fc1_dims, w.fc2_dims = 23, 400, 300
    return w


def weights_of(net):
    cached = getattr(net, "_tt_weights", None)
    key = tuple(p.data_ptr() for p in net.parameters())
    if cached is not None and cached[0] == key:
        return cached[1]
    w = _fill_weights(net, L.TTMlpWeights())
    net._tt_split_ws = torch.empty(int(L.load().tt_mlp_split_ws_bytes()), dtype=torch.uint8, device=net.fc2.weight.device)
    w.split_ws = net._tt_split_ws.data_ptr()
    net._tt_weights = (key, w)
    return w


def packed_weights_of(net, index, max_workgroups=None, capped_grids=None, two_images=None):
    cache = net.__dict__.setdefault("_tt_packed", {})
    key = tuple(p.data_ptr() for p in net.parameters())
    hit = cache.get(index)
    if hit is None or hit[0] != key:
        old = hit[1] if hit is not None else None
        w = _fill_weights(net, L.TTMlpWeights())
        ws = torch.empty(int(L.load().tt_mlp_split_ws_bytes()), dtype=torch.uint8, device=net.fc2.weight.device)
        w.split_ws, w.ws_packed = ws.data_ptr(), 1
        hit = cache[index] = (key, w, ws)
        if old is not None:
            w.max_workgroups, w.capped_grids = old.max_workgroups, old.capped_grids
            two_images = two_images or bool(old.split_ws_alt)
    if max_workgroups is not None:
        hit[1].max_workgroups = int(max_workgroups)
    if capped_grids is not None:
        hit[1].capped_grids = int(capped_grids)
    if two_images and not hit[1].split_ws_alt:
        alt = torch.empty(int(L.load().tt_mlp_split_ws_bytes()), dtype=torch.uint8, device=net.fc2.weight.device)
        hit[1].split_ws_alt = alt.data_ptr()
        cache[index] = hit + (alt,)
    return hit[1]


def packed_key_of(net):
    return tuple(p.data_ptr() for p in net.parameters())


def pack(net, index, bump=None, cursor=None):
    w = packed_weights_of(net, index)
    dev = net.fc2.weight.device
    L.check(L.load().tt_mlp_split_pack(C.byref(w), 1 if hasattr(net, "action_value") else 0, C.c_void_p(w.split_ws),
                                       L.ptr(bump), C.byref(cursor) if cursor is not None else None,
                                       L.stream(dev)))


@contextlib.contextmanager
def exact_f32(net):
    w = weights_of(net)
    ws, w.split_ws = w.split_ws, None
    try:
        yield
    finally:
        w.split_ws = ws


def _stream(t):
    return L.stream(t.device)


def actor_forward(net, obs, out=None):
    n = obs.shape[0]
    out = torch.empty(n, dtype=torch.float32, device=obs.device) if out is None else out
    L.check(L.load().tt_actor_forward(n, L.ptr(obs), C.byref(weights_of(net)), L.ptr(out), _stream(obs)))
    return out.view(n, 1)


def critic_forward(net, obs, action, out=None):
    n = obs.shape[0]
    out = torch.empty(n, dtype=torch.float32, device=obs.device) if out is None else out
    L.check(L.load().tt_critic_forward(n, L.ptr(obs), L.ptr(action), C.byref(weights_of(net)), L.ptr(out), _stream(obs)))
    return out.view(n, 1)


def actor_act(net, obs, ou_state, act_raw, act_scaled, seed, step=0, step_dev=None, done_prev=None, mu_out=None,
              theta=0.2, sigma=0.15, dt=1e-2, high=math.pi / 4, weights=None):
    n = obs.shape[0]
    L.check(L.load().tt_actor_act(n, L.ptr(obs), C.byref(weights if weights is not None else weights_of(net)), L.ptr(ou_state), L.ptr(done_prev),
                                  int(seed) & (2 ** 64 - 1), int(step), L.ptr(step_dev), float(theta * dt),
                                  float(sigma * math.sqrt(dt)), float(high), L.ptr(mu_out), L.ptr(act_raw),
                                  L.ptr(act_scaled), _stream(obs)))
    return act_scaled


def policy_kernel_info(n):
    waves = 4 * ((n + 127) // 128)
    return {"kernel": "k_mlp_split (choose_action for N envs; split-f16; the image's pack launch, ~4 us per step, not included)",
            "mfma_flop": waves * (750 + 78) * 32768.0,
            "note": "f16 MFMA FLOP executed (three f16 products per f32 product block, both layers) over the dense f16/bf16 "
                    "peak; algorithmic_* = the network's useful f32 FLOP"}
```

### include/ttenv.h

```cpp
#ifndef TTENV_H
#define TTENV_H

#include <stddef.h>
#include <stdint.h>

#ifdef __cplusplus
extern "C" {
#endif

#define TT_VERSION 3
#define TT_OBS_DIM 23
#define TT_MAX_EPISODE_STEPS 4095

enum { TT_OK = 0, TT_EINVAL = -1, TT_ENOMEM = -2, TT_EHIP = -3, TT_ENODEV = -4 };

enum {
    TT_F_JACKKNIFE = 1, TT_F_OUT_OF_MAP = 2, TT_F_MAX_STEPS = 4, TT_F_GOAL_REACHED = 8,
    TT_F_GOAL_PASSED = 16, TT_F_EXCESSIVE_BACK = 32, TT_F_SUCCESS = 64
};
#define TT_TERM_SIMV2 0x3F
#define TT_TERM_SIMV1 0x0F

enum {
    TT_V_NONE = 0, TT_V_JACKKNIFE, TT_V_JACKKNIFE_WARNING, TT_V_MAJOR_BOUNDARY, TT_V_MINOR_BOUNDARY,
    TT_V_PAST_THE_GOAL, TT_V_MAX_STEP, TT_V_EXCESSIVE_BACKWARD
};

enum {
    TT_I_TOTAL = 0, TT_I_PROGRESS, TT_I_HEADING, TT_I_ORIENT, TT_I_STAGED, TT_I_SAFETY, TT_I_EXPLORE,
    TT_I_FINAL, TT_I_BACKWARD, TT_I_SMOOTH, TT_I_CUMBACK, TT_I_BUDGET, TT_NINFO
};

typedef struct ihipStream_t *tt_stream_t;
typedef struct tt_env tt_env;

typedef struct tt_params {
    double L1, L2;
    double hitch_offset, v1x;
    double dt;
    double map_min_x, map_max_x, map_min_y, map_max_y;
    double max_steer;
    double position_threshold, orientation_threshold;
    double step_length;
    int32_t extra_steps;
    int32_t fixed_max_steps;
    uint32_t term_mask;
    int32_t variant;
    int32_t stateless_reward;
    int32_t reserved_;
    double goal[3];
    double reset_lo[3], reset_hi[3];
} tt_params;

typedef struct tt_info {
    double *comp;
    uint8_t *violation;
    uint8_t *flags;
} tt_info;

int tt_version(void);
const char *tt_last_error(const tt_env *env);

int tt_params_default(int variant, tt_params *out);

int tt_env_create(int n_envs, int device, const tt_params *params, tt_env **out);
int tt_env_destroy(tt_env *env);
int tt_env_num_envs(const tt_env *env);

int tt_env_reset(tt_env *env, const uint8_t *mask, uint64_t seed, float *obs_out, tt_stream_t stream);

int tt_env_set_reset_pool(tt_env *env, const double *pool, int m);

int tt_env_set_pose(tt_env *env, const int32_t *idx, int k, const double *start ,
                    const double *goal , const double *L2 , float *obs_out,
                    tt_stream_t stream);

int tt_env_set_attrs(tt_env *env, const int32_t *idx, int k, const double *start ,
                     const double *goal , const double *L2 , tt_stream_t stream);

int tt_env_set_state(tt_env *env, const int32_t *idx, int k, const double *state, tt_stream_t stream);
int tt_env_get_state(tt_env *env, double *state_out, tt_stream_t stream);

int tt_env_set_max_steps(tt_env *env, const int32_t *idx, int k, const int32_t *max_steps, tt_stream_t stream);

int tt_env_set_steps(tt_env *env, const int32_t *idx, int k, const int32_t *steps, tt_stream_t stream);

int tt_env_get_episode(tt_env *env, int32_t *steps, int32_t *max_steps, double *start, double *goal, double *L2,
                       tt_stream_t stream);

int tt_env_observe(tt_env *env, const float *steering, float *obs_out, tt_stream_t stream);

int tt_env_set_step_counter(tt_env *env, int64_t *counter);

int tt_env_step(tt_env *env, const float *action, float *obs, float *reward, uint8_t *done, const tt_info *info,
                int auto_reset, tt_stream_t stream);

typedef struct tt_ring_view {
    int32_t *cursor;
    float *obs, *act, *rew;
    uint8_t *done;
    int32_t n_envs, slots;
} tt_ring_view;
typedef struct tt_ring_cursor {
    const int64_t *k_dev;
    int32_t slots, reserved_;
    int32_t *cursor;
} tt_ring_cursor;
#define TT_CURSOR_INTS 32
#define TT_CURSOR_GAVE_UP 15
#define TT_CURSOR_GAVE_UP_MIRROR 18
#define TT_CURSOR_PROGRESS 16
int tt_env_step_ring(tt_env *env, const float *action, const tt_ring_view *ring, int auto_reset, tt_stream_t stream);

int tt_env_step_random(tt_env *env, uint64_t policy_seed, float *action_out, float *obs, float *reward,
                       uint8_t *done, const tt_info *info, int auto_reset, tt_stream_t stream);

size_t tt_env_state_bytes(const tt_env *env);
int tt_env_export(tt_env *env, void *blob, uint64_t meta[4], tt_stream_t stream);
int tt_env_import(tt_env *env, const void *blob, const uint64_t meta[4], tt_stream_t stream);

#define TT_LOG_NCOUNTS 9
int tt_env_set_episode_log(tt_env *env, int64_t capacity, tt_stream_t stream);
int tt_env_drain_episode_log(tt_env *env, double *ret, int32_t *len, uint8_t *flags, uint8_t *success, int32_t *lane,
                             int64_t *end_step, int64_t *n_out, uint64_t *counts_out, tt_stream_t stream);
size_t tt_env_episode_log_bytes(const tt_env *env);
int tt_env_export_episode_log(tt_env *env, void *blob, uint64_t meta[2], tt_stream_t stream);
int tt_env_import_episode_log(tt_env *env, const void *blob, const uint64_t meta[2], tt_stream_t stream);

#define TT_LOG_DETAIL 1
#define TT_LOG_NCOMP 9
int tt_env_set_episode_log2(tt_env *env, int64_t capacity, uint32_t flags, tt_stream_t stream);
int tt_env_drain_episode_log2(tt_env *env, double *ret, int32_t *len, uint8_t *flags, uint8_t *success, int32_t *lane,
                              int64_t *end_step, double *comp, double *start, int64_t *n_out, uint64_t *counts_out,
                              tt_stream_t stream);

int tt_env_rollout_random(tt_env *env, int k_steps, uint64_t policy_seed, float *obs_out, float *reward_sum,
                          int32_t *episodes_done, tt_stream_t stream);

int tt_env_profile(tt_env *env, int max_launches);
int tt_env_profile_read(tt_env *env, double *total_ms, int64_t *launches);

int tt_random_actions(int n, uint64_t seed, uint64_t step, float *out, tt_stream_t stream);

typedef struct tt_mlp_weights {
    const float *w1, *b1, *g1, *be1, *w2, *b2, *g2, *be2, *w3, *b3, *wa, *ba;
    int32_t in_dim, fc1_dims, fc2_dims;
    int32_t capped_grids;
    void *split_ws;
    int32_t ws_packed;
    int32_t max_workgroups;
    void *split_ws_alt;
    void *fc2_img;
} tt_mlp_weights;
uint64_t tt_mlp_fc2_image_bytes(void);
int tt_mlp_fc2_image_pack(const tt_mlp_weights *w, tt_stream_t stream);
typedef struct tt_fc2_images {
    void *net, *target;
} tt_fc2_images;
uint64_t tt_mlp_split_ws_bytes(void);
int tt_mlp_split_pack(const tt_mlp_weights *w, int critic, void *ws, int64_t *bump, const tt_ring_cursor *cursor,
                      tt_stream_t stream);

int tt_actor_forward(int n, const float *obs , const tt_mlp_weights *w, float *mu_out, tt_stream_t stream);

int tt_actor_act(int n, const float *obs, const tt_mlp_weights *w, float *ou_state, const uint8_t *done_prev,
                 uint64_t seed, uint64_t step, const int64_t *step_dev, float theta_dt, float sigma_sqrt_dt, float high,
                 float *mu_out, float *act_raw_out, float *act_scaled_out, tt_stream_t stream);

int tt_actor_act_ring(int n, const tt_ring_view *ring, const tt_mlp_weights *w, float *ou_state, uint64_t seed, uint64_t step,
                      const int64_t *step_dev, float theta_dt, float sigma_sqrt_dt, float high, float *act_scaled_out,
                      tt_stream_t stream);

typedef struct tt_side_buffer {
    const float *obs, *act, *rew, *obs2;
    const uint8_t *done;
    int32_t count, reserved_;
} tt_side_buffer;
int tt_ring_sample(int batch, int n_envs, int slots, const int64_t *k_dev, const float *obs, const float *act,
                   const float *rew, const uint8_t *done, uint64_t seed, int reserve, int lag, const tt_side_buffer *side,
                   float *s_out, float *a_out, float *r_out, float *s2_out, uint8_t *d_out, int32_t *idx_out,
                   tt_stream_t stream);

typedef struct tt_sample_args {
    int32_t batch, n_envs, slots, reserve;
    const int64_t *k_dev;
    const float *obs, *act, *rew;
    const uint8_t *done;
    uint64_t seed;
    const tt_side_buffer *side;
    float *s_out, *a_out, *r_out, *s2_out;
    uint8_t *d_out;
    int32_t *idx_out;
    int32_t lag;
    int32_t draws;
    uint64_t seed_stride;
    const int32_t *step_progress;
} tt_sample_args;
int tt_mlp_split_pack_and_sample(const tt_mlp_weights *w, int critic, void *ws, const tt_sample_args *sample,
                                 const tt_ring_cursor *cursor, tt_stream_t stream);

int tt_critic_forward(int n, const float *obs , const float *action , const tt_mlp_weights *w,
                      float *q_out, tt_stream_t stream);

typedef struct tt_mlp_saved {
    float *xh1, *h1;
    float *xh2, *h2;
    float *rstd1, *rstd2;
} tt_mlp_saved;

int tt_mlp_forward_save(int n, int critic, const float *obs, const float *action, const tt_mlp_weights *w, float *out,
                        const tt_mlp_saved *saved, float *dq_da, tt_stream_t stream);

typedef struct tt_fwd_job {
    int32_t critic, reserved_;
    const float *obs, *action;
    const tt_mlp_weights *w;
    float *out;
    const tt_mlp_saved *saved;
    float *dq_da, *z_state;
} tt_fwd_job;
int tt_mlp_forward_multi(int n, int count, const tt_fwd_job *jobs, tt_stream_t stream);
int tt_mlp_forward_multi_sampled(int n, int count, const tt_fwd_job *jobs, const tt_sample_args *sample, int64_t *k_snapshot,
                                 tt_stream_t stream);

#define TT_NSTEP_MAX 16
int tt_ring_sample_nstep(const tt_sample_args *sample, int n_step, float gamma, tt_stream_t stream);
int tt_mlp_forward_multi_sampled_nstep(int n, int count, const tt_fwd_job *jobs, const tt_sample_args *sample, int n_step,
                                       float gamma, int64_t *k_snapshot, tt_stream_t stream);

typedef struct tt_mlp_bwd_ws {
    float *dpre, *dz, *dx2, *dy1, *dx1;
} tt_mlp_bwd_ws;
typedef struct tt_td_input {
    const float *z_state, *mu_target;
    const tt_mlp_weights *target_critic;
    const float *reward;
    const uint8_t *done;
    float gamma, reserved_;
    float *y_out, *q_out;
    int64_t *step_dev;
    int64_t *window_dev;
    float *bias_corr_out;
    float adam_beta1, adam_beta2;
} tt_td_input;
#define TT_BIAS_CORR_FLOATS 8

typedef struct tt_image_job {
    const tt_mlp_weights *actor;
    const tt_ring_cursor *cursor;
} tt_image_job;
int tt_mlp_backward_rows_pair(int n, float scale_critic, const float *q_out, const tt_mlp_weights *critic,
                              const tt_mlp_saved *saved_critic, const tt_mlp_bwd_ws *ws_critic, const tt_td_input *td,
                              const float *mu_out, const tt_mlp_weights *actor, const tt_mlp_saved *saved_actor,
                              const tt_mlp_bwd_ws *ws_actor, const tt_image_job *image, tt_stream_t stream);
int tt_mlp_backward_weights(int n, int critic, const float *obs, const float *action, const tt_mlp_saved *saved,
                            const tt_mlp_bwd_ws *ws, const tt_mlp_weights *grads, const float *row_dq_da, const float *row_mu,
                            float row_scale, int count, float *const *params, float *const *exp_avg, float *const *exp_avg_sq,
                            float *const *targets, const int64_t *step_dev, float lr, float beta1, float beta2, float eps,
                            float weight_decay, float tau, const tt_fc2_images *images ,
                            const float *bias_corr , tt_stream_t stream);

int tt_mlp_actor_tail(int n, const float *obs, const float *mu, const tt_mlp_weights *critic, float *q_out, float *dq_da,
                      const tt_mlp_saved *saved, const tt_mlp_bwd_ws *ws, const tt_mlp_weights *grads, float row_scale, int count,
                      float *const *params, float *const *exp_avg, float *const *exp_avg_sq, float *const *targets,
                      const int64_t *step_dev, float lr, float beta1, float beta2, float eps, float weight_decay, float tau,
                      const tt_fc2_images *images, const float *bias_corr, int32_t *tail_words, int32_t *gave_up_host,
                      tt_stream_t stream);

int tt_adam_soft_update(int count, float *const *params, const float *const *grads, float *const *exp_avg,
                        float *const *exp_avg_sq, float *const *targets, const int32_t *numel, const int64_t *step_dev,
                        float lr, float beta1, float beta2, float eps, float weight_decay, float tau,
                        const tt_fc2_images *images ,
                        const float *bias_corr , tt_stream_t stream);

#define TT_POP_MAX_AGENTS 16
typedef struct tt_population tt_population;
typedef struct tt_pop_net {
    const tt_mlp_bwd_ws *ws;
    const tt_mlp_weights *grads;
    int32_t count, reserved_;
    float *const *params, *const *exp_avg, *const *exp_avg_sq, *const *targets;
    float lr, beta1, beta2, eps, weight_decay, tau;
    const tt_fc2_images *images;
} tt_pop_net;
typedef struct tt_pop_agent {
    const tt_sample_args *sample;
    const tt_fwd_job *jobs;
    const tt_td_input *td;
    tt_pop_net critic, actor;
    float *q_pi, *dq_da;
    int32_t *tail_words, *gave_up_host;
} tt_pop_agent;
int tt_pop_learn_create(int count, int batch, const tt_pop_agent *agents , tt_population **out);
int tt_pop_learn(tt_population *pop, int update, tt_stream_t stream);
int tt_pop_learn_destroy(tt_population *pop);

typedef struct tt_pop_exploit_pair {
    int32_t dst, src;
    float alpha, beta, tau, gamma;
} tt_pop_exploit_pair;
int tt_pop_exploit(tt_population *pop, int pairs, const tt_pop_exploit_pair *list , tt_stream_t stream);
int tt_pop_hyper(tt_population *pop, int agent, float out[4]);

struct tt_pop_nstep {
    int32_t n_step;
    float gamma, discount;
};
int tt_pop_learn_set_nstep(tt_population *pop, const struct tt_pop_nstep *per_agent );
int tt_pop_exploit_nstep(tt_population *pop, int pairs, const tt_pop_exploit_pair *list ,
                         const struct tt_pop_nstep *ns , tt_stream_t stream);
int tt_pop_nstep(tt_population *pop, int agent, struct tt_pop_nstep *out);

#define TT_LEARN_LOG_NVALUES 16
#define TT_LEARN_LOG_CHUNKS 16
#define TT_LEARN_LOG_MAX_CAPACITY (1 << 22)
typedef struct tt_learn_log tt_learn_log;
typedef struct tt_learn_log_job {
    const float *y, *q, *q_pi, *dq_da, *mu;
    const float *grad_critic, *grad_actor;
    int32_t numel_critic, numel_actor;
    const int64_t *step_dev;
} tt_learn_log_job;
int tt_learn_log_create(int agents, int batch, const tt_learn_log_job *jobs , int64_t capacity, int32_t every,
                        tt_learn_log **out);
int tt_learn_log_append(tt_learn_log *log, tt_stream_t stream);
int tt_learn_log_drain(tt_learn_log *log, int agent, int64_t after_step, int64_t max, int64_t *step_out, double *values_out,
                       int32_t *nonfinite_out, int64_t *count);
int tt_learn_log_clear(tt_learn_log *log, tt_stream_t stream);
int tt_learn_log_destroy(tt_learn_log *log);

typedef struct tt_p2p tt_p2p;
#define TT_P2P_MAX_RANKS 8
#define TT_P2P_MAX_SITES 4
#define TT_P2P_HANDLE_BYTES 128
int tt_p2p_create(int device, int rank, int world, int sites, const int32_t *numel , tt_p2p **out);
int tt_p2p_destroy(tt_p2p *x);
int tt_p2p_export(const tt_p2p *x, void *handle_out );
int tt_p2p_attach(tt_p2p *x, int peer, const void *handle );
float *tt_p2p_grad(const tt_p2p *x, int site);
int tt_p2p_reset(tt_p2p *x, tt_stream_t stream);
int tt_p2p_set_timeout(tt_p2p *x, double seconds);
int tt_p2p_gave_up(const tt_p2p *x);
const char *tt_p2p_last_error(const tt_p2p *x);
int tt_adam_soft_update_p2p(tt_p2p *x, int site, int count, float *const *params, float *const *exp_avg,
                            float *const *exp_avg_sq, float *const *targets, const int32_t *numel, const int64_t *step_dev,
                            float lr, float beta1, float beta2, float eps, float weight_decay, float tau,
                            const tt_fc2_images *images, const float *bias_corr, tt_stream_t stream);

typedef struct tt_td3 tt_td3;
typedef struct tt_td3_agent {
    const tt_sample_args *sample;
    const tt_fwd_job *jobs;
    const tt_td_input *td;
    tt_pop_net critic, critic_2, actor;
    const float *z_state_2;
    const tt_mlp_weights *target_critic_2;
    float target_noise, noise_clip;
    uint64_t noise_seed;
    float *eps_out, *y2_out, *q2t_out;
    int64_t *step_snapshot, *actor_step_dev;
    float *actor_bias_corr_out;
    float *q_pi, *dq_da;
    int32_t *tail_words, *gave_up_host;
} tt_td3_agent;
int tt_td3_create(int batch, const tt_td3_agent *agent, tt_td3 **out);
int tt_td3_update(tt_td3 *h, const tt_td3_agent *agent);
int tt_td3_learn(tt_td3 *h, int update, int full, tt_stream_t stream);
int tt_td3_destroy(tt_td3 *h);

typedef struct tt_pop_td3 tt_pop_td3;
typedef struct tt_pop_td3_pair {
    int32_t dst, src;
    float alpha, beta, tau, gamma, target_noise, noise_clip;
} tt_pop_td3_pair;
int tt_pop_td3_create(int count, int batch, const tt_td3_agent *agents , tt_pop_td3 **out);
int tt_pop_td3_learn(tt_pop_td3 *pop, int update, int full, tt_stream_t stream);
int tt_pop_td3_exploit(tt_pop_td3 *pop, int pairs, const tt_pop_td3_pair *list , tt_stream_t stream);
int tt_pop_td3_hyper(tt_pop_td3 *pop, int agent, float out[6]);
int tt_pop_td3_destroy(tt_pop_td3 *pop);

#ifdef __cplusplus
}
#endif
#endif
```

Before: 833.7 million.

## Add alternate split-MLP schedule overlapping next tile's obs loads and RNG with layer 2

Moves the kernel body into a shared header and builds a second schedule variant, k_mlp_split_shadow. This variant spreads the next tile's observation loads and OU-noise RNG pieces across free slots of the layer-2 MFMA issue schedule, and interleaves the layer-2 bias/LayerNorm pass with the MFMAs. Compile-time checks recompute the counted vmcnt waits. A runtime setter selects between the schedules. The aim is to hide per-tile load and RNG latency, at the cost of higher register pressure and more complex wait accounting.

```diff
diff --git a/ddpg-trucktrailer_amd/_lib.py b/ddpg-trucktrailer_amd/_lib.py
--- a/ddpg-trucktrailer_amd/_lib.py
+++ b/ddpg-trucktrailer_amd/_lib.py
@@ -179,6 +179,7 @@
     "tt_env_profile": (C.c_int, [_P, _I]),
     "tt_env_profile_read": (C.c_int, [_P, C.POINTER(C.c_double), C.POINTER(C.c_int64)]),
     "tt_mlp_split_ws_bytes": (C.c_uint64, []),
+    "tt_mlp_split_schedule_set": (C.c_int, [_I]),
     "tt_mlp_split_pack": (C.c_int, [C.POINTER(TTMlpWeights), _I, _P, _P, C.POINTER(TTRingCursor), _P]),
     "tt_mlp_split_pack_and_sample": (C.c_int, [C.POINTER(TTMlpWeights), _I, _P, C.POINTER(TTSampleArgs), C.POINTER(TTRingCursor), _P]),
     "tt_actor_act_ring": (C.c_int, [_I, C.POINTER(TTRingView), C.POINTER(TTMlpWeights), _P, _U64, _U64, _P, C.c_float, C.c_float,
diff --git a/ddpg-trucktrailer_amd/build.py b/ddpg-trucktrailer_amd/build.py
--- a/ddpg-trucktrailer_amd/build.py
+++ b/ddpg-trucktrailer_amd/build.py
@@ -5,7 +5,7 @@
 HERE = os.path.dirname(os.path.abspath(__file__))
 ROOT = os.path.dirname(HERE)
 SRC = [os.path.join(HERE, "csrc", f) for f in ("ttenv.hip", "ttnet.hip", "ttnet_split.hip", "ttlearn.hip", "ttp2p.hip", "ttpop.hip", "ttnstep.hip", "ttpop_nstep.hip", "ttlearnlog.hip", "tttd3.hip", "ttpop_td3.hip")]
-HDR = [os.path.join(ROOT, "include", "ttenv.h"), os.path.join(HERE, "csrc", "ttnet_common.h"), os.path.join(HERE, "csrc", "ttnet_pack.h"), os.path.join(HERE, "csrc", "ttp2p.h"), os.path.join(HERE, "csrc", "ttstamps.h"), os.path.join(HERE, "csrc", "ttlearn_bodies.h"), os.path.join(HERE, "csrc", "ttnstep.h"), os.path.join(HERE, "csrc", "ttpop.h"), os.path.join(HERE, "csrc", "tthost.h"), os.path.join(HERE, "csrc", "ttphilox.h"), os.path.join(HERE, "csrc", "tttd3.h")]
+HDR = [os.path.join(ROOT, "include", "ttenv.h"), os.path.join(HERE, "csrc", "ttnet_common.h"), os.path.join(HERE, "csrc", "ttnet_pack.h"), os.path.join(HERE, "csrc", "ttnet_split_kernel.h"), os.path.join(HERE, "csrc", "ttp2p.h"), os.path.join(HERE, "csrc", "ttstamps.h"), os.path.join(HERE, "csrc", "ttlearn_bodies.h"), os.path.join(HERE, "csrc", "ttnstep.h"), os.path.join(HERE, "csrc", "ttpop.h"), os.path.join(HERE, "csrc", "tthost.h"), os.path.join(HERE, "csrc", "ttphilox.h"), os.path.join(HERE, "csrc", "tttd3.h")]
 LIB = os.path.join(HERE, "libttenv.so")
 
 
diff --git a/ddpg-trucktrailer_amd/csrc/ttnet.hip b/ddpg-trucktrailer_amd/csrc/ttnet.hip
--- a/ddpg-trucktrailer_amd/csrc/ttnet.hip
+++ b/ddpg-trucktrailer_amd/csrc/ttnet.hip
@@ -261,6 +261,7 @@
 #endif
 
 uint64_t tt_mlp_split_ws_bytes(void) { return (uint64_t)split_ws_bytes(); }
+int tt_mlp_split_schedule_set(int schedule) { return split_schedule_set(schedule); }
 
 static RingCursor to_cursor(const tt_ring_cursor *c) {
     return (c && c->cursor && c->k_dev && c->slots > 0)
diff --git a/ddpg-trucktrailer_amd/csrc/ttnet_common.h b/ddpg-trucktrailer_amd/csrc/ttnet_common.h
--- a/ddpg-trucktrailer_amd/csrc/ttnet_common.h
+++ b/ddpg-trucktrailer_amd/csrc/ttnet_common.h
@@ -290,6 +290,7 @@
 }
 
 size_t split_ws_bytes();
+int split_schedule_set(int schedule);
 int split_pack(const tt_mlp_weights *w, bool critic, void *ws, long long *bump, const RingCursor &cur, hipStream_t stream);
 int split_pack_and_sample(const tt_mlp_weights *w, bool critic, void *ws, const RingSample &R, const RingCursor &cur,
                           hipStream_t stream);
diff --git a/ddpg-trucktrailer_amd/csrc/ttnet_split.hip b/ddpg-trucktrailer_amd/csrc/ttnet_split.hip
--- a/ddpg-trucktrailer_amd/csrc/ttnet_split.hip
+++ b/ddpg-trucktrailer_amd/csrc/ttnet_split.hip
@@ -1,3 +1,5 @@
+#include <cstdlib>
+
 #include "ttnet_common.h"
 #include "ttnet_pack.h"
 #include "ttstamps.h"
@@ -40,6 +42,10 @@
 }
 
 constexpr int JOB_NONE = -1, JOB_FC1 = 100, JOB_NEXT = 200;
+constexpr int JOB_OBS = 300, OBS_FEATURES = 15, OBS_STEP0 = 14;
+constexpr int obs_loads(const bool critic) { return OBS_FEATURES + (critic ? 0 : 2); }
+constexpr int JOB_RNG = 400, RNG_PIECES = 24;
+constexpr bool job_is_vm(const int j) { return j != JOB_NONE && j < JOB_RNG; }
 constexpr int TAIL0 = STEPS - (RING - 1);
 constexpr int l2_job(const int s, const int u) {
     if (s == 0) return AHEAD - 1 + u / 5;
@@ -51,6 +57,14 @@
     if (s == TAIL0 + 3 || s == TAIL0 + 4) return JOB_NEXT + s - (TAIL0 + 3);
     return JOB_NONE;
 }
+constexpr int l2_job(const int loads, const int s, const int u) {
+    const int j = l2_job(s, u);
+    if (j != JOB_NONE || u >= 5 || s < OBS_STEP0) return j;
+    const int i = 5 * (s - OBS_STEP0) + u;
+    if (loads == 0) return JOB_NONE;
+    return i < loads ? JOB_OBS + i : (i < loads + RNG_PIECES ? JOB_RNG + i - loads : JOB_NONE);
+}
+static_assert(5 * (STEPS - 1 - OBS_STEP0) >= obs_loads(false) + RNG_PIECES, "the next tile's loads and sample do not fit the free slots");
 constexpr int l2_piece(const int u) { return u % 5; }
 constexpr int job_slot(const int j) { return j >= JOB_NEXT ? j - JOB_NEXT : (j >= JOB_FC1 ? W1_OFF / CHUNK_BYTES + (j - JOB_FC1) / 5 : j % RING); }
 constexpr bool l2_slots_free() {
@@ -58,39 +72,74 @@
         for (int u = 0; u < T2; ++u) {
             const int j = l2_job(s, u);
             if (j == JOB_NONE) continue;
+            if (l2_job(obs_loads(false), s, u) != j) return false;
             if (s == 0 || (s == 1 && u < 5)) { if (job_slot(j) < W1_OFF / CHUNK_BYTES) return false; }
             else if (u < 5 || job_slot(j) != (s - 1) % RING) return false;
         }
     return true;
 }
 static_assert(l2_slots_free(), "a piece of layer 2 overwrites a slot that may still be read");
-constexpr int mid_allowed(const int s) {
+constexpr int mid_allowed(const int loads, const int s) {
     int n = 10, after = s + 1 == 2 ? 5 : (s + 1 == 3 ? 10 : -1000);
     for (int ss = 0; ss < STEPS; ++ss)
         for (int u = 0; u < T2; ++u) {
             if (ss == s && u == T2 / 2) return n - after;
-            const int j = l2_job(ss, u);
-            if (j != JOB_NONE) { ++n; if (j == s + 1) after = n; }
+            const int j = l2_job(loads, ss, u);
+            if (job_is_vm(j)) { ++n; if (j == s + 1) after = n; }
         }
     return -1;
 }
+constexpr int mid_allowed(const int s) { return mid_allowed(0, s); }
 constexpr bool mid_counts_ok() {
     for (int s = 1; s + 1 < STEPS; ++s) if (mid_allowed(s) != (s < TAIL0 + 3 ? 20 : 18)) return false;
     return true;
 }
 static_assert(mid_counts_ok(), "the counted waits of layer 2 do not match the issue schedule");
+constexpr int obs_loads_before_mid(const int loads, const int s) {
+    int n = 0;
+    for (int ss = 0; ss <= s; ++ss)
+        for (int u = 0; u < T2 / 2; ++u) if (l2_job(loads, ss, u) >= JOB_OBS && l2_job(loads, ss, u) < JOB_RNG) ++n;
+    return n;
+}
+constexpr bool mid_counts1_ok(const int loads) {
+    int total = 0;
+    for (int s = 0; s < STEPS; ++s)
+        for (int u = 0; u < T2; ++u)
+            if (l2_job(loads, s, u) >= JOB_OBS && l2_job(loads, s, u) < JOB_RNG) { if (u >= T2 / 2 || l2_job(loads, s, u) != JOB_OBS + total) return false; ++total; }
+    if (total != loads) return false;
+    for (int s = 1; s + 1 < STEPS; ++s) {
+        const int younger = obs_loads_before_mid(loads, s) - (s >= 5 ? obs_loads_before_mid(loads, s - 5) : 0);
+        if (mid_allowed(loads, s) != mid_allowed(0, s) + younger || mid_allowed(loads, s) > 63) return false;
+    }
+    return true;
+}
+static_assert(mid_counts1_ok(obs_loads(false)) && mid_counts1_ok(obs_loads(true)), "the counted waits of schedule 1 do not match its issue schedule");
 struct L2Schedule {
     int job[STEPS][T2], mid[STEPS];
 };
-constexpr L2Schedule make_l2_schedule() {
+constexpr L2Schedule make_l2_schedule(const int loads = 0) {
     L2Schedule t{};
     for (int s = 0; s < STEPS; ++s) {
-        t.mid[s] = mid_allowed(s);
-        for (int u = 0; u < T2; ++u) t.job[s][u] = l2_job(s, u);
+        t.mid[s] = mid_allowed(loads, s);
+        for (int u = 0; u < T2; ++u) t.job[s][u] = l2_job(loads, s, u);
     }
     return t;
 }
 constexpr L2Schedule L2S = make_l2_schedule();
+constexpr L2Schedule L2S1[2] = {make_l2_schedule(obs_loads(false)), make_l2_schedule(obs_loads(true))};
+#define TT_MID_CASES(X) X(18) X(20) X(22) X(25) X(27) X(30) X(32) X(35) X(37)
+constexpr bool mid_has_case(const int m) {
+#define TT_MID_IS(c) if (m == c) return true;
+    TT_MID_CASES(TT_MID_IS)
+#undef TT_MID_IS
+    return false;
+}
+constexpr bool mid_cases_ok() {
+    for (int c = 0; c < 2; ++c)
+        for (int s = 1; s + 1 < STEPS; ++s) if (!mid_has_case(L2S1[c].mid[s])) return false;
+    return true;
+}
+static_assert(mid_cases_ok(), "a counted wait of schedule 1 has no case in the kernel text");
 
 using lds_b = const __attribute__((address_space(3))) unsigned char;
 using v4u = __attribute__((ext_vector_type(4))) unsigned;
@@ -103,387 +152,32 @@
     return make_uint4(t[0], t[1], t[2], t[3]);
 }
 
-template <bool CRITIC>
-__global__ __launch_bounds__(256, 1) void k_mlp_split(const int n, const int tile0, const int tile_end,
-                                                      int *__restrict__ cursor_e, const long long *__restrict__ step_e,
-                                                      const float *__restrict__ obs,
-                                                      const unsigned char *__restrict__ ws,
-                                                      const unsigned char *__restrict__ ws_alt,
-                                                      const float *__restrict__ action, float *__restrict__ out,
-                                                      const ActArgs act) {
-    extern __shared__ __attribute__((aligned(16))) unsigned char lds_raw[];
-    const float *p1_s = reinterpret_cast<const float *>(lds_raw + RING_BYTES);
-    const int tid = threadIdx.x, lane = tid & 63;
-    const int wave = __builtin_amdgcn_readfirstlane(tid >> 6);
-    const int r = lane & 31, h = lane >> 5;
-    using lds_f = const __attribute__((address_space(3))) float;
-    using v4 = __attribute__((ext_vector_type(4))) float;
-    auto lds4 = [](lds_f *q) -> float4 {
-        const v4 t = *(const __attribute__((address_space(3))) v4 *)q;
-        return make_float4(t[0], t[1], t[2], t[3]);
-    };
-    lds_f *pv1_0 = (lds_f *)(p1_s + 4 * h);
-    LdsBases LB0;
-    LB0.b0 = (lds_b *)lds_raw + lane * 16;
-    LB0.b1 = LB0.b0 + 65536;
-    LB0.b2 = LB0.b0 + 131072;
-    const EpochPair epochs = await_image_early(cursor_e);
-    const long long kstep = cursor_e ? *step_e : 0;
-    const bool odd = act.cursor && (kstep & 1);
-    const bool local = act.cursor && act.ring_slots > 0;
-    const int slot_t = !local ? 0 : ((unsigned long long)kstep >> 32) == 0ull ? (int)((unsigned)kstep % (unsigned)act.ring_slots)
-                                                                             : (int)(kstep % act.ring_slots);
-    const float *obs_base = local ? obs + (size_t)slot_t * act.ring_n * IN : obs;
-    const unsigned lds_base0 = (unsigned)(uintptr_t)(__attribute__((address_space(3))) unsigned char *)lds_raw;
-    auto dma_piece = [&](const unsigned char *base, const unsigned voff, const unsigned lds_wave, const unsigned dst_const)
-                         __attribute__((always_inline)) {
-        unsigned keep;
-        asm volatile("s_mov_b32 %0, m0\n\ts_add_u32 m0, %3, %4\n\ts_nop 0\n\tglobal_load_lds_dwordx4 %1, %2\n\ts_mov_b32 m0, %0"
-                     : "=&s"(keep) : "v"(voff), "s"(base), "s"(lds_wave), "s"(dst_const) : "memory", "scc");
-    };
-    const unsigned voff_w2 = lane * 16 + wave * 5120 + WS_W2;
-    const unsigned voff_w1 = lane * 16 + wave * 1024 + WS_W1;
-    const unsigned voff_vec = lane * 16 + wave * (VEC_PIECES / 4) * 1024 + WS_VEC;
-    const unsigned ldsw_w2_0 = lds_base0 + wave * 5120, ldsw_w1_0 = lds_base0 + W1_OFF + wave * 1024;
-    auto issue_fc1_piece = [&](const unsigned char *w, const unsigned ldsw_w1, const int i) __attribute__((always_inline)) {
-        dma_piece(w, voff_w1 + i * 4096, ldsw_w1, i * 4096);
-    };
-    auto issue_step_piece = [&](const unsigned char *w, const unsigned ldsw_w2, const int s, const int i) __attribute__((always_inline)) {
-        dma_piece(w, voff_w2 + s * CHUNK_BYTES + i * 1024, ldsw_w2, (s % RING) * CHUNK_BYTES + i * 1024);
-    };
-    float xo[S1][8];
-    float ou_pre = 0.f;
-    unsigned dp_pre = 0u;
-    const bool with_noise = !CRITIC && act.ou != nullptr;
-    const uint8_t *dprev = act.done_prev;
-    float *araw = act.act_raw;
-    auto load_obs = [&](const int tile) __attribute__((always_inline)) {
-        const int row = tile * ROWS + wave * WROWS + r;
-        const int rowc = row < n ? row : n - 1;
-        const float *orow = obs_base + (size_t)rowc * IN;
-#pragma unroll
-        for (int s = 0; s < S1; ++s)
-#pragma unroll
-            for (int j = 0; j < 8; ++j) {
-                const int k = 16 * s + 8 * h + j;
-                xo[s][j] = orow[k < IN ? k : IN - 1];
-            }
-        if (with_noise) {
-            ou_pre = act.ou[rowc];
-            dp_pre = dprev ? (unsigned)dprev[rowc] : 0u;
-        }
-    };
-
-    NSTAMP(0);
-    int tile = tile0 + (int)blockIdx.x;
-    if (tile >= tile_end) return;
-    if (local) {
-        const int sl = act.ring_slots;
-        const int slot_prev = slot_t == 0 ? sl - 1 : slot_t - 1;
-        dprev = kstep > 0 ? act.done_prev + (size_t)slot_prev * act.ring_n : nullptr;
-        araw = act.act_raw + (size_t)slot_t * act.ring_n;
-    }
-    if (!act.cursor || local) load_obs(tile);
-    await_image(act.cursor, act.step_dev, epochs);
-    const unsigned char *wsl = (odd && ws_alt) ? ws_alt : ws;
-    if (act.cursor && !local) {
-        obs_base = resolve_obs(act, obs);
-        const int *c = cursor_of(act);
-        dprev = c[3] ? act.done_prev + (size_t)c[2] * act.ring_n : nullptr;
-        araw = act.act_raw + (size_t)c[0] * act.ring_n;
-        load_obs(tile);
-    }
-    const unsigned long long noise_step = act.step + (act.step_dev ? (unsigned long long)*act.step_dev : 0ull);
-    if (act.cursor && tile0 == 0 && blockIdx.x == 0 && tid == 0)
-        __hip_atomic_store(act.cursor + CUR_PROGRESS, (int)(kstep + 1), __ATOMIC_RELAXED, __HIP_MEMORY_SCOPE_AGENT);
-    if (act.cursor && tile0 == 0 && blockIdx.x == 0 && tid < 4) {
-        const int sl = act.ring_slots;
-        act.cursor[tid] = !local ? cursor_of(act)[tid]
-                                 : (tid == 0 ? slot_t : tid == 1 ? (slot_t + 1 == sl ? 0 : slot_t + 1)
-                                                      : tid == 2 ? (slot_t == 0 ? sl - 1 : slot_t - 1) : (kstep > 0 ? 1 : 0));
-    }
-#pragma unroll
-    for (int i = 0; i < W1_WAVE_PIECES; ++i) issue_fc1_piece(wsl, ldsw_w1_0, i);
-#pragma unroll
-    for (int i = 0; i < VEC_PIECES / 4; ++i)
-        dma_piece(wsl, voff_vec + i * 1024, lds_base0 + RING_BYTES + wave * (VEC_PIECES / 4) * 1024, i * 1024);
-    bool first = true;
-#ifdef TT_STAMPS
-    int round = 0;
-    if (threadIdx.x == 0 && blockIdx.x < 512) for (int q = 0; q < 4; ++q) g_tile[blockIdx.x][q][0] = g_tile[blockIdx.x][q][1] = 0ull;
-    if (threadIdx.x == 0 && blockIdx.x < 512) g_tile[blockIdx.x][0][0] = wall_clock64();
-#endif
-
-#pragma unroll 1
-    for (;;) {
-        const unsigned char *wsl_cur = wsl;
-        unsigned ldsw_w2 = ldsw_w2_0, ldsw_w1 = ldsw_w1_0;
-        LdsBases LB = LB0;
-        lds_f *pv1 = pv1_0;
-        asm volatile("" : "+s"(wsl_cur), "+s"(ldsw_w2), "+s"(ldsw_w1), "+v"(LB.b0), "+v"(LB.b1), "+v"(LB.b2), "+v"(pv1));
-        lds_f *pv2 = pv1 + 2 * H1P;
-        const int row = tile * ROWS + wave * WROWS + r;
-#pragma unroll
-        for (int s = 0; s < S1; ++s)
-#pragma unroll
-            for (int j = 0; j < 8; ++j) {
-                const int k = 16 * s + 8 * h + j;
-                xo[s][j] = k < IN ? (row < n ? xo[s][j] : 0.f) : (k == IN ? 1.f : 0.f);
-            }
-        float ou_next = 0.f;
-        if (with_noise) ou_next = ou_advance(row < n ? row : n - 1, ou_pre, dp_pre != 0u, act, noise_step);
-        uint4 xb[S1][2];
-#pragma unroll
-        for (int s = 0; s < S1; ++s) {
-            uint32_t ph[4], pm[4];
-#pragma unroll
-            for (int p = 0; p < 4; ++p) split2(xo[s][2 * p] * SX, xo[s][2 * p + 1] * SX, ph[p], pm[p]);
-            xb[s][0] = make_uint4(ph[0], ph[1], ph[2], ph[3]);
-            xb[s][1] = make_uint4(pm[0], pm[1], pm[2], pm[3]);
-        }
-        asm volatile("s_waitcnt vmcnt(0)" ::: "memory");
-        __builtin_amdgcn_s_barrier();
-        if (first) NSTAMP(1);
-
-#define SB __builtin_amdgcn_sched_barrier(0)
-        f32x16 acc1[T1];
-        {
-            auto w1_frag = [&](const int q, const int plane) __attribute__((always_inline)) {
-                return lds_frag(LB, W1_OFF + (((q % S1) * T1 + q / S1) * 2 + plane) * 1024);
-            };
-            const unsigned char *wsl_1 = wsl_cur;
-            asm volatile("" : "+s"(wsl_1));
-            uint4 a0h = w1_frag(0, 0), a0m = w1_frag(0, 1), a1h = w1_frag(1, 0), a1m = w1_frag(1, 1), a2h = a0h, a2m = a0m;
-            SB;
-#pragma unroll
-            for (int q = 0; q < S1 * T1; ++q) {
-                const int t = q / S1, s = q % S1;
-                if (s == 0) {
-#pragma unroll
-                    for (int v = 0; v < 16; ++v) acc1[t][v] = 0.f;
-                }
-                acc1[t] = mfma_f16(a0m, xb[s][0], acc1[t]); SB;
-                if (q + 2 < S1 * T1) a2h = w1_frag(q + 2, 0);
-                SB;
-                acc1[t] = mfma_f16(a0h, xb[s][1], acc1[t]); SB;
-                if (q + 2 < S1 * T1) a2m = w1_frag(q + 2, 1);
-                SB;
-                acc1[t] = mfma_f16(a0h, xb[s][0], acc1[t]); SB;
-                if (q < 10) { if (first) issue_step_piece(wsl_1, ldsw_w2, q / 5, q % 5); }
-                else if (q < 20) issue_step_piece(wsl_1, ldsw_w2, 2 + (q - 10) / 5, q % 5);
-                SB;
-                a0h = a1h; a0m = a1m; a1h = a2h; a1m = a2m;
-            }
-        }
-        if (first) NSTAMP(2);
-        uint32_t hb[STEPS][4], mb[STEPS][4];
-        f32x2 nmean, rstdp;
-        {
-            f32x2 sp = pk(0.f, 0.f);
-#pragma unroll
-            for (int t = 0; t < T1; ++t)
-#pragma unroll
-                for (int v = 0; v < (t == T1 - 1 ? 8 : 16); v += 4)
-                    sp += pk(acc1[t][v], acc1[t][v + 1]) + pk(acc1[t][v + 2], acc1[t][v + 3]);
-            const float s = sp[0] + sp[1];
-            const float mean = (s + __shfl_xor(s, 32)) * (1.f / H1);
-            nmean = pk(-mean, -mean);
-            f32x2 ssp = pk(0.f, 0.f);
-#pragma unroll
-            for (int t = 0; t < T1; ++t)
-#pragma unroll
-                for (int v = 0; v < (t == T1 - 1 ? 8 : 16); v += 2) {
-                    const f32x2 d = pk(acc1[t][v], acc1[t][v + 1]) + nmean;
-                    ssp = pk_fma(d, d, ssp);
-                }
-            const float ss = ssp[0] + ssp[1];
-            const float var = (ss + __shfl_xor(ss, 32)) * (1.f / H1) * (UNSCALE * UNSCALE);
-            const float rstd = rsqrtf(var + 1e-5f) * UNSCALE;
-            rstdp = pk(rstd, rstd);
-        }
-        constexpr int GROUPS = 2 * STEPS;
-        float4 gq[2], bq[2];
-        f32x2 ya, yb;
-        float y0, y1, y2, y3;
-        auto ln_read = [&](const int G) __attribute__((always_inline)) {
-            gq[G & 1] = lds4(pv1 + 8 * G);
-            bq[G & 1] = lds4(pv1 + H1P + 8 * G);
-        };
-        auto ln_chunk = [&](const int G, const int k) __attribute__((always_inline)) {
-            const int t = G >> 2, i = G & 3, st = G >> 1, e = 2 * (G & 1);
-            const float4 g = gq[G & 1], be = bq[G & 1];
-            if (k == 0) ya = pk_fma((pk(acc1[t][4 * i], acc1[t][4 * i + 1]) + nmean) * rstdp, pk(g.x, g.y), pk(be.x, be.y));
-            if (k == 1) yb = pk_fma((pk(acc1[t][4 * i + 2], acc1[t][4 * i + 3]) + nmean) * rstdp, pk(g.z, g.w), pk(be.z, be.w));
-            if (k == 2) {
-                y0 = fmaxf(ya[0], 0.f); y1 = fmaxf(ya[1], 0.f); y2 = fmaxf(yb[0], 0.f); y3 = fmaxf(yb[1], 0.f);
-                if (G + 1 < GROUPS) ln_read(G + 1);
-            }
-            if (k == 3) split2(y0, y1, hb[st][e], mb[st][e]);
-            if (k == 4) split2(y2, y3, hb[st][e + 1], mb[st][e + 1]);
-        };
-        ln_read(0);
-#pragma unroll
-        for (int G = 0; G < 4; ++G)
-#pragma unroll
-            for (int k = 0; k < 5; ++k) ln_chunk(G, k);
-
-        if (first) NSTAMP(3);
-        f32x16 acc2[T2];
-#pragma unroll
-        for (int u = 0; u < T2; ++u)
-#pragma unroll
-            for (int v = 0; v < 16; ++v) acc2[u][v] = 0.f;
-        asm volatile("s_waitcnt vmcnt(10)" ::: "memory");
-        __builtin_amdgcn_s_barrier();
-        uint4 c0h = lds_frag(LB, 0), c0m = lds_frag(LB, 1024), c1h = lds_frag(LB, 2048), c1m = lds_frag(LB, 3072), c2h = c0h, c2m = c0m;
-        SB;
-        auto l2_step = [&](const int s) __attribute__((always_inline)) {
-            const uint4 vh = make_uint4(hb[s][0], hb[s][1], hb[s][2], hb[s][3]), vm = make_uint4(mb[s][0], mb[s][1], mb[s][2], mb[s][3]);
-            const int slot = (s % RING) * CHUNK_BYTES, nslot = ((s + 1) % RING) * CHUNK_BYTES;
-            const unsigned char *wsl_s = wsl_cur;
-            unsigned lds_s = ldsw_w2, lds1_s = ldsw_w1;
-            asm volatile("" : "+s"(wsl_s), "+s"(lds_s));
-            if (s >= TAIL0 && s < TAIL0 + 3) asm volatile("" : "+s"(lds1_s));
-#pragma unroll
-            for (int u = 0; u < T2; ++u) {
-                if (u == T2 / 2 && s >= 1 && s + 1 < STEPS) {
-                    switch (L2S.mid[s]) {
-                        case 20: asm volatile("s_waitcnt vmcnt(20)" ::: "memory"); break;
-                        default: asm volatile("s_waitcnt vmcnt(18)" ::: "memory"); break;
-                    }
-                    __builtin_amdgcn_s_barrier();
-                    SB;
-                }
-                const bool more = u + 2 < T2 || s + 1 < STEPS;
-                const int nx = u + 2 < T2 ? slot + (u + 2) * 2048 : nslot + (u + 2 - T2) * 2048;
-                acc2[u] = mfma_f16(c0h, vm, acc2[u]); SB;
-                if (more) c2h = lds_frag(LB, nx);
-                if (s + 2 < STEPS) ln_chunk(2 * (s + 2) + u / 5, u % 5);
-                SB;
-                acc2[u] = mfma_f16(c0m, vh, acc2[u]); SB;
-                if (more) c2m = lds_frag(LB, nx + 1024);
-                SB;
-                acc2[u] = mfma_f16(c0h, vh, acc2[u]); SB;
-                {
-                    const int j = L2S.job[s][u];
-                    const bool f1 = j >= JOB_FC1 && j < JOB_NEXT;
-                    const int st = j >= JOB_NEXT ? j - JOB_NEXT : j, i1 = j - JOB_FC1;
-                    if (j != JOB_NONE)
-                        dma_piece(wsl_s, f1 ? voff_w1 + i1 * 4096 : voff_w2 + st * CHUNK_BYTES + l2_piece(u) * 1024, f1 ? lds1_s : lds_s,
-                                  f1 ? i1 * 4096 : (st % RING) * CHUNK_BYTES + l2_piece(u) * 1024);
-                }
-                SB;
-                c0h = c1h; c0m = c1m; c1h = c2h; c1m = c2m;
-            }
-        };
-#pragma unroll
-        for (int s = 0; s < 2; ++s) l2_step(s);
-#pragma unroll
-        for (int s = 2; s < TAIL0; ++s) l2_step(s);
-#pragma unroll
-        for (int s = TAIL0; s < STEPS; ++s) l2_step(s);
-#undef SB
-
-        if (first) NSTAMP(4);
-        const int next = tile + (int)gridDim.x;
-        const bool more_tiles = next < tile_end;
-        if (more_tiles) load_obs(next);
-        f32x2 s2p = pk(0.f, 0.f);
-        {
-            float4 bq[2][4];
-            auto ldb = [&](const int u, float4 (&b)[4]) {
-#pragma unroll
-                for (int i = 0; i < 4; ++i) b[i] = lds4(pv2 + 32 * u + 8 * i);
-            };
-            ldb(0, bq[0]);
-#pragma unroll
-            for (int u = 0; u < T2; ++u) {
-                if (u + 1 < T2) ldb(u + 1, bq[(u + 1) & 1]);
-                __builtin_amdgcn_sched_barrier(0);
-#pragma unroll
-                for (int i = 0; i < 4; ++i) {
-                    const float4 b = bq[u & 1][i];
-                    const f32x2 xa = pk_fma(pk(acc2[u][4 * i], acc2[u][4 * i + 1]), pk(UNSCALE, UNSCALE), pk(b.x, b.y));
-                    const f32x2 xb2 = pk_fma(pk(acc2[u][4 * i + 2], acc2[u][4 * i + 3]), pk(UNSCALE, UNSCALE), pk(b.z, b.w));
-                    acc2[u][4 * i] = xa[0]; acc2[u][4 * i + 1] = xa[1]; acc2[u][4 * i + 2] = xb2[0]; acc2[u][4 * i + 3] = xb2[1];
-                    s2p += xa + xb2;
-                }
-                __builtin_amdgcn_sched_barrier(0);
-            }
-        }
-        const float s2 = s2p[0] + s2p[1];
-        const float mean2 = (s2 + __shfl_xor(s2, 32)) * (1.f / H2);
-        const f32x2 nmean2 = pk(-mean2, -mean2);
-        f32x2 ss2p = pk(0.f, 0.f);
-#pragma unroll
-        for (int u = 0; u < T2; ++u)
-#pragma unroll
-            for (int i = 0; i < 4; ++i) {
-                const bool real = 32 * u + 8 * i + 4 * h < H2;
-                const f32x2 keep = real ? pk(1.f, 1.f) : pk(0.f, 0.f);
-#pragma unroll
-                for (int j = 0; j < 4; j += 2) {
-                    const f32x2 d = pk(acc2[u][4 * i + j], acc2[u][4 * i + j + 1]) + nmean2;
-                    acc2[u][4 * i + j] = d[0]; acc2[u][4 * i + j + 1] = d[1];
-                    const f32x2 dk = (32 * u + 8 * i + 4 < H2) ? d : d * keep;
-                    ss2p = pk_fma(dk, dk, ss2p);
-                }
-            }
-        const float ss2 = ss2p[0] + ss2p[1];
-        const float rstd2 = rsqrtf((ss2 + __shfl_xor(ss2, 32)) * (1.f / H2) + 1e-5f);
-        const f32x2 rstd2p = pk(rstd2, rstd2);
-        const float av = (CRITIC && row < n) ? action[row] : 0.f;
-        f32x2 dotp = pk(0.f, 0.f);
-        {
-            constexpr int NV = CRITIC ? 5 : 3;
-            float4 vq[2][4][NV];
-            auto ldv = [&](const int u, float4 (&v)[4][NV]) {
-#pragma unroll
-                for (int i = 0; i < 4; ++i)
-#pragma unroll
-                    for (int q = 0; q < NV; ++q) v[i][q] = lds4(pv2 + (q + 1) * H2P + 32 * u + 8 * i);
-            };
-            ldv(0, vq[0]);
-#pragma unroll
-            for (int u = 0; u < T2; ++u) {
-                if (u + 1 < T2) ldv(u + 1, vq[(u + 1) & 1]);
-                __builtin_amdgcn_sched_barrier(0);
-#pragma unroll
-                for (int i = 0; i < 4; ++i) {
-                    const float4 g = vq[u & 1][i][0], be = vq[u & 1][i][1], w3 = vq[u & 1][i][2];
-                    f32x2 ya = pk_fma(pk(acc2[u][4 * i], acc2[u][4 * i + 1]) * rstd2p, pk(g.x, g.y), pk(be.x, be.y));
-                    f32x2 yb = pk_fma(pk(acc2[u][4 * i + 2], acc2[u][4 * i + 3]) * rstd2p, pk(g.z, g.w), pk(be.z, be.w));
-                    if (CRITIC) {
-                        const float4 wa = vq[u & 1][i][NV - 2], ba = vq[u & 1][i][NV - 1];
-                        ya += pk_fma(pk(av, av), pk(wa.x, wa.y), pk(ba.x, ba.y));
-                        yb += pk_fma(pk(av, av), pk(wa.z, wa.w), pk(ba.z, ba.w));
-                    }
-                    dotp = pk_fma(pk(fmaxf(ya[0], 0.f), fmaxf(ya[1], 0.f)), pk(w3.x, w3.y), dotp);
-                    dotp = pk_fma(pk(fmaxf(yb[0], 0.f), fmaxf(yb[1], 0.f)), pk(w3.z, w3.w), dotp);
-                }
-                __builtin_amdgcn_sched_barrier(0);
-            }
-        }
-        const float dot = dotp[0] + dotp[1];
-        const float v = dot + __shfl_xor(dot, 32) + lds4(pv1 - 4 * h + VEC_FLOATS).x;
-        if (h == 0 && row < n) {
-            if (with_noise) finish_row_noise(row, v, out, act, ou_next, araw);
-            else finish_row<CRITIC>(row, v, out, act);
-        }
-        if (first) NSTAMP(5);
-#ifdef TT_STAMPS
-        TSTAMP(round, 1);
-        if (threadIdx.x == 0 && blockIdx.x < 512 && round < 4) tt_log_add(g_log_tile, g_tile[blockIdx.x][round][0], g_tile[blockIdx.x][round][1]);
-        ++round;
-        if (more_tiles) TSTAMP(round, 0);
-#endif
-        if (!more_tiles) break;
-        tile = next;
-        first = false;
-    }
-    asm volatile("s_waitcnt vmcnt(0)" ::: "memory");
-}
-
+#define TT_SPLIT_KERNEL k_mlp_split
+#define TT_SPLIT_SCHED 0
+#include "ttnet_split_kernel.h"
+#undef TT_SPLIT_KERNEL
+#undef TT_SPLIT_SCHED
+#define TT_SPLIT_KERNEL k_mlp_split_shadow
+#define TT_SPLIT_SCHED 1
+#include "ttnet_split_kernel.h"
+#undef TT_SPLIT_KERNEL
+#undef TT_SPLIT_SCHED
+
+int g_schedule = -1;
+int schedule_now() {
+    if (g_schedule < 0) {
+        const char *e = getenv("TT_POLICY_SCHEDULE");
+        g_schedule = (e && e[0] == '1') ? 1 : 0;
+    }
+    return g_schedule;
+}
+
+}
+
+int split_schedule_set(int schedule) {
+    const int prev = schedule_now();
+    if (schedule == 0 || schedule == 1) g_schedule = schedule;
+    return prev;
 }
 
 #ifdef TT_STAMPS
@@ -530,8 +224,11 @@
     static int cus[64] = {};
     int dev = 0;
     if (hipGetDevice(&dev) != hipSuccess || dev < 0 || dev >= 64) return TT_EHIP;
+    const auto kernel = schedule_now() ? &k_mlp_split_shadow<CRITIC> : &k_mlp_split<CRITIC>;
     if (!attr[dev]) {
         if (hipFuncSetAttribute(reinterpret_cast<const void *>(&k_mlp_split<CRITIC>),
+                                hipFuncAttributeMaxDynamicSharedMemorySize, LDS_BYTES) != hipSuccess ||
+            hipFuncSetAttribute(reinterpret_cast<const void *>(&k_mlp_split_shadow<CRITIC>),
                                 hipFuncAttributeMaxDynamicSharedMemorySize, LDS_BYTES) != hipSuccess)
             return TT_EHIP;
         int c = 0;
@@ -547,13 +244,13 @@
         capped = ntiles;
         if (w->capped_grids > 0 && (long long)w->capped_grids * limit < ntiles) capped = w->capped_grids * limit;
         const int rounds = (capped + limit - 1) / limit, g = (capped + rounds - 1) / rounds;
-        hipLaunchKernelGGL((k_mlp_split<CRITIC>), dim3(g), dim3(256), LDS_BYTES, stream, n, 0, capped, act.cursor, act.step_dev, obs,
+        hipLaunchKernelGGL(kernel, dim3(g), dim3(256), LDS_BYTES, stream, n, 0, capped, act.cursor, act.step_dev, obs,
                            reinterpret_cast<const unsigned char *>(w->split_ws),
                            reinterpret_cast<const unsigned char *>(w->split_ws_alt), action, out, act);
     }
     if (capped < ntiles) {
         const int rest = ntiles - capped, rounds = (rest + chip - 1) / chip, g = (rest + rounds - 1) / rounds;
-        hipLaunchKernelGGL((k_mlp_split<CRITIC>), dim3(g), dim3(256), LDS_BYTES, stream, n, capped, ntiles, act.cursor, act.step_dev, obs,
+        hipLaunchKernelGGL(kernel, dim3(g), dim3(256), LDS_BYTES, stream, n, capped, ntiles, act.cursor, act.step_dev, obs,
                            reinterpret_cast<const unsigned char *>(w->split_ws),
                            reinterpret_cast<const unsigned char *>(w->split_ws_alt), action, out, act);
     }
diff --git a/ddpg-trucktrailer_amd/csrc/ttnet_split_kernel.h b/ddpg-trucktrailer_amd/csrc/ttnet_split_kernel.h
--- /dev/null
+++ b/ddpg-trucktrailer_amd/csrc/ttnet_split_kernel.h
@@ -0,0 +1,518 @@
+
+template <bool CRITIC>
+__global__ __launch_bounds__(256, 1) void TT_SPLIT_KERNEL(const int n, const int tile0, const int tile_end,
+                                                          int *__restrict__ cursor_e, const long long *__restrict__ step_e,
+                                                          const float *__restrict__ obs,
+                                                          const unsigned char *__restrict__ ws,
+                                                          const unsigned char *__restrict__ ws_alt,
+                                                          const float *__restrict__ action, float *__restrict__ out,
+                                                          const ActArgs act) {
+    extern __shared__ __attribute__((aligned(16))) unsigned char lds_raw[];
+    const float *p1_s = reinterpret_cast<const float *>(lds_raw + RING_BYTES);
+    const int tid = threadIdx.x, lane = tid & 63;
+    const int wave = __builtin_amdgcn_readfirstlane(tid >> 6);
+    const int r = lane & 31, h = lane >> 5;
+    using lds_f = const __attribute__((address_space(3))) float;
+    using v4 = __attribute__((ext_vector_type(4))) float;
+    auto lds4 = [](lds_f *q) -> float4 {
+        const v4 t = *(const __attribute__((address_space(3))) v4 *)q;
+        return make_float4(t[0], t[1], t[2], t[3]);
+    };
+    lds_f *pv1_0 = (lds_f *)(p1_s + 4 * h);
+    LdsBases LB0;
+    LB0.b0 = (lds_b *)lds_raw + lane * 16;
+    LB0.b1 = LB0.b0 + 65536;
+    LB0.b2 = LB0.b0 + 131072;
+    const EpochPair epochs = await_image_early(cursor_e);
+    const long long kstep = cursor_e ? *step_e : 0;
+    const bool odd = act.cursor && (kstep & 1);
+    const bool local = act.cursor && act.ring_slots > 0;
+    const int slot_t = !local ? 0 : ((unsigned long long)kstep >> 32) == 0ull ? (int)((unsigned)kstep % (unsigned)act.ring_slots)
+                                                                             : (int)(kstep % act.ring_slots);
+    const float *obs_base = local ? obs + (size_t)slot_t * act.ring_n * IN : obs;
+    const unsigned lds_base0 = (unsigned)(uintptr_t)(__attribute__((address_space(3))) unsigned char *)lds_raw;
+    auto dma_piece = [&](const unsigned char *base, const unsigned voff, const unsigned lds_wave, const unsigned dst_const)
+                         __attribute__((always_inline)) {
+        unsigned keep;
+        asm volatile("s_mov_b32 %0, m0\n\ts_add_u32 m0, %3, %4\n\ts_nop 0\n\tglobal_load_lds_dwordx4 %1, %2\n\ts_mov_b32 m0, %0"
+                     : "=&s"(keep) : "v"(voff), "s"(base), "s"(lds_wave), "s"(dst_const) : "memory", "scc");
+    };
+    const unsigned voff_w2 = lane * 16 + wave * 5120 + WS_W2;
+    const unsigned voff_w1 = lane * 16 + wave * 1024 + WS_W1;
+    const unsigned voff_vec = lane * 16 + wave * (VEC_PIECES / 4) * 1024 + WS_VEC;
+    const unsigned ldsw_w2_0 = lds_base0 + wave * 5120, ldsw_w1_0 = lds_base0 + W1_OFF + wave * 1024;
+    auto issue_fc1_piece = [&](const unsigned char *w, const unsigned ldsw_w1, const int i) __attribute__((always_inline)) {
+        dma_piece(w, voff_w1 + i * 4096, ldsw_w1, i * 4096);
+    };
+    auto issue_step_piece = [&](const unsigned char *w, const unsigned ldsw_w2, const int s, const int i) __attribute__((always_inline)) {
+        dma_piece(w, voff_w2 + s * CHUNK_BYTES + i * 1024, ldsw_w2, (s % RING) * CHUNK_BYTES + i * 1024);
+    };
+    float xo[S1][8];
+    float ou_pre = 0.f;
+    unsigned dp_pre = 0u;
+    const bool with_noise = !CRITIC && act.ou != nullptr;
+    const uint8_t *dprev = act.done_prev;
+    float *araw = act.act_raw;
+    auto load_obs = [&](const int tile) __attribute__((always_inline)) {
+        const int row = tile * ROWS + wave * WROWS + r;
+        const int rowc = row < n ? row : n - 1;
+        const float *orow = obs_base + (size_t)rowc * IN;
+#pragma unroll
+        for (int s = 0; s < S1; ++s)
+#pragma unroll
+            for (int j = 0; j < 8; ++j) {
+                const int k = 16 * s + 8 * h + j;
+                xo[s][j] = orow[k < IN ? k : IN - 1];
+            }
+        if (with_noise) {
+            ou_pre = act.ou[rowc];
+            dp_pre = dprev ? (unsigned)dprev[rowc] : 0u;
+        }
+    };
+
+#if TT_SPLIT_SCHED == 1
+    auto load_next = [&](const int tile_now, const int i) __attribute__((always_inline)) {
+        const int row = (tile_now + (int)gridDim.x) * ROWS + wave * WROWS + r;
+        const int rowc = row < n ? row : n - 1;
+        if (i < OBS_FEATURES) {
+            const int k = 16 * (i / 8) + 8 * h + i % 8;
+            int kc = k < IN ? k : IN - 1;
+            asm volatile("" : "+v"(kc));
+            xo[i / 8][i % 8] = (obs_base + (size_t)rowc * IN)[kc];
+        } else if (i == OBS_FEATURES) {
+            ou_pre = (with_noise ? act.ou : obs_base)[rowc];
+        } else {
+            dp_pre = (unsigned)(with_noise && dprev ? dprev : reinterpret_cast<const uint8_t *>(obs_base))[rowc];
+        }
+    };
+    static_assert(OBS_FEATURES == IN - 8 && S1 == 2, "the schedule's load jobs: the features of the inputs below IN for h = 0");
+#endif
+    NSTAMP(0);
+    int tile = tile0 + (int)blockIdx.x;
+    if (tile >= tile_end) return;
+    if (local) {
+        const int sl = act.ring_slots;
+        const int slot_prev = slot_t == 0 ? sl - 1 : slot_t - 1;
+        dprev = kstep > 0 ? act.done_prev + (size_t)slot_prev * act.ring_n : nullptr;
+        araw = act.act_raw + (size_t)slot_t * act.ring_n;
+    }
+    if (!act.cursor || local) load_obs(tile);
+    await_image(act.cursor, act.step_dev, epochs);
+    const unsigned char *wsl = (odd && ws_alt) ? ws_alt : ws;
+    if (act.cursor && !local) {
+        obs_base = resolve_obs(act, obs);
+        const int *c = cursor_of(act);
+        dprev = c[3] ? act.done_prev + (size_t)c[2] * act.ring_n : nullptr;
+        araw = act.act_raw + (size_t)c[0] * act.ring_n;
+        load_obs(tile);
+    }
+    const unsigned long long noise_step = act.step + (act.step_dev ? (unsigned long long)*act.step_dev : 0ull);
+#if TT_SPLIT_SCHED == 1
+    float nrm_pre = 0.f;
+    uint32_t pc0 = 0u, pc1 = 0u, pc2 = 0u, pc3 = 0u, pn2 = 0u, plo0 = 0u;
+    float pu1 = 0.f, pu2 = 0.f, pln = 0.f, psq = 0.f;
+    auto rng_piece = [&](const int tile_now, const int i) __attribute__((always_inline)) {
+        if (i < 20) {
+            const int rd = i >> 1;
+            if (i == 0) {
+                const int row = (tile_now + (int)gridDim.x) * ROWS + wave * WROWS + r;
+                pc0 = (uint32_t)(row < n ? row : n - 1); pc1 = (uint32_t)noise_step; pc2 = (uint32_t)(noise_step >> 32); pc3 = 0x0A5Eu;
+            }
+            if ((i & 1) == 0) {
+                pn2 = __umulhi(0xD2511F53u, pc0) ^ pc3 ^ ((uint32_t)(act.seed >> 32) + (uint32_t)rd * 0xBB67AE85u);
+                plo0 = 0xD2511F53u * pc0;
+            } else {
+                const uint32_t hi1 = __umulhi(0xCD9E8D57u, pc2), lo1 = 0xCD9E8D57u * pc2;
+                pc0 = hi1 ^ pc1 ^ ((uint32_t)act.seed + (uint32_t)rd * 0x9E3779B9u); pc1 = lo1; pc2 = pn2; pc3 = plo0;
+            }
+        } else if (i == 20) {
+            pu1 = ((float)(pc0 >> 8) + 0.5f) * (1.f / 16777216.f);
+            pu2 = ((float)(pc1 >> 8) + 0.5f) * (1.f / 16777216.f);
+        } else if (i == 21) {
+            pln = logf(pu1);
+        } else if (i == 22) {
+            psq = sqrtf(-2.f * pln);
+        } else {
+            nrm_pre = psq * cosf(6.28318530717958647692f * pu2);
+        }
+    };
+    static_assert(RNG_PIECES == 24, "20 half rounds, the uniforms, logf, sqrtf, cosf");
+#endif
+    if (act.cursor && tile0 == 0 && blockIdx.x == 0 && tid == 0)
+        __hip_atomic_store(act.cursor + CUR_PROGRESS, (int)(kstep + 1), __ATOMIC_RELAXED, __HIP_MEMORY_SCOPE_AGENT);
+    if (act.cursor && tile0 == 0 && blockIdx.x == 0 && tid < 4) {
+        const int sl = act.ring_slots;
+        act.cursor[tid] = !local ? cursor_of(act)[tid]
+                                 : (tid == 0 ? slot_t : tid == 1 ? (slot_t + 1 == sl ? 0 : slot_t + 1)
+                                                      : tid == 2 ? (slot_t == 0 ? sl - 1 : slot_t - 1) : (kstep > 0 ? 1 : 0));
+    }
+#pragma unroll
+    for (int i = 0; i < W1_WAVE_PIECES; ++i) issue_fc1_piece(wsl, ldsw_w1_0, i);
+#pragma unroll
+    for (int i = 0; i < VEC_PIECES / 4; ++i)
+        dma_piece(wsl, voff_vec + i * 1024, lds_base0 + RING_BYTES + wave * (VEC_PIECES / 4) * 1024, i * 1024);
+    bool first = true;
+#ifdef TT_STAMPS
+    int round = 0;
+    if (threadIdx.x == 0 && blockIdx.x < 512) for (int q = 0; q < 4; ++q) g_tile[blockIdx.x][q][0] = g_tile[blockIdx.x][q][1] = 0ull;
+    if (threadIdx.x == 0 && blockIdx.x < 512) g_tile[blockIdx.x][0][0] = wall_clock64();
+#endif
+
+#pragma unroll 1
+    for (;;) {
+        const unsigned char *wsl_cur = wsl;
+        unsigned ldsw_w2 = ldsw_w2_0, ldsw_w1 = ldsw_w1_0;
+        LdsBases LB = LB0;
+        lds_f *pv1 = pv1_0;
+        asm volatile("" : "+s"(wsl_cur), "+s"(ldsw_w2), "+s"(ldsw_w1), "+v"(LB.b0), "+v"(LB.b1), "+v"(LB.b2), "+v"(pv1));
+        lds_f *pv2 = pv1 + 2 * H1P;
+        const int row = tile * ROWS + wave * WROWS + r;
+#pragma unroll
+        for (int s = 0; s < S1; ++s)
+#pragma unroll
+            for (int j = 0; j < 8; ++j) {
+                const int k = 16 * s + 8 * h + j;
+                xo[s][j] = k < IN ? (row < n ? xo[s][j] : 0.f) : (k == IN ? 1.f : 0.f);
+            }
+        float ou_next = 0.f;
+#if TT_SPLIT_SCHED == 1
+        if (with_noise) {
+            const bool restart = (first || dprev != nullptr) && dp_pre != 0u;
+            if (first) ou_next = ou_advance(row < n ? row : n - 1, ou_pre, restart, act, noise_step);
+            else ou_next = fmaf(restart ? 0.f : ou_pre, act.decay, act.scale * nrm_pre);
+        }
+#else
+        if (with_noise) ou_next = ou_advance(row < n ? row : n - 1, ou_pre, dp_pre != 0u, act, noise_step);
+#endif
+        uint4 xb[S1][2];
+#pragma unroll
+        for (int s = 0; s < S1; ++s) {
+            uint32_t ph[4], pm[4];
+#pragma unroll
+            for (int p = 0; p < 4; ++p) split2(xo[s][2 * p] * SX, xo[s][2 * p + 1] * SX, ph[p], pm[p]);
+            xb[s][0] = make_uint4(ph[0], ph[1], ph[2], ph[3]);
+            xb[s][1] = make_uint4(pm[0], pm[1], pm[2], pm[3]);
+        }
+        asm volatile("s_waitcnt vmcnt(0)" ::: "memory");
+        __builtin_amdgcn_s_barrier();
+        if (first) NSTAMP(1);
+
+#define SB __builtin_amdgcn_sched_barrier(0)
+        f32x16 acc1[T1];
+#if TT_SPLIT_SCHED == 1
+        f32x2 sp1 = pk(0.f, 0.f);
+        auto ln1_sum = [&](const int t, const int v) __attribute__((always_inline)) {
+            sp1 += pk(acc1[t][v], acc1[t][v + 1]) + pk(acc1[t][v + 2], acc1[t][v + 3]);
+        };
+#endif
+        {
+            auto w1_frag = [&](const int q, const int plane) __attribute__((always_inline)) {
+                return lds_frag(LB, W1_OFF + (((q % S1) * T1 + q / S1) * 2 + plane) * 1024);
+            };
+            const unsigned char *wsl_1 = wsl_cur;
+            asm volatile("" : "+s"(wsl_1));
+            uint4 a0h = w1_frag(0, 0), a0m = w1_frag(0, 1), a1h = w1_frag(1, 0), a1m = w1_frag(1, 1), a2h = a0h, a2m = a0m;
+            SB;
+#pragma unroll
+            for (int q = 0; q < S1 * T1; ++q) {
+                const int t = q / S1, s = q % S1;
+                if (s == 0) {
+#pragma unroll
+                    for (int v = 0; v < 16; ++v) acc1[t][v] = 0.f;
+                }
+                acc1[t] = mfma_f16(a0m, xb[s][0], acc1[t]); SB;
+                if (q + 2 < S1 * T1) a2h = w1_frag(q + 2, 0);
+#if TT_SPLIT_SCHED == 1
+                if (t > 0) ln1_sum(t - 1, 8 * s);
+#endif
+                SB;
+                acc1[t] = mfma_f16(a0h, xb[s][1], acc1[t]); SB;
+                if (q + 2 < S1 * T1) a2m = w1_frag(q + 2, 1);
+#if TT_SPLIT_SCHED == 1
+                if (t > 0) ln1_sum(t - 1, 8 * s + 4);
+#endif
+                SB;
+                acc1[t] = mfma_f16(a0h, xb[s][0], acc1[t]); SB;
+                if (q < 10) { if (first) issue_step_piece(wsl_1, ldsw_w2, q / 5, q % 5); }
+                else if (q < 20) issue_step_piece(wsl_1, ldsw_w2, 2 + (q - 10) / 5, q % 5);
+                SB;
+                a0h = a1h; a0m = a1m; a1h = a2h; a1m = a2m;
+            }
+        }
+        if (first) NSTAMP(2);
+        uint32_t hb[STEPS][4], mb[STEPS][4];
+        f32x2 nmean, rstdp;
+        {
+            f32x2 sp = pk(0.f, 0.f);
+#if TT_SPLIT_SCHED == 1
+            ln1_sum(T1 - 1, 0);
+            ln1_sum(T1 - 1, 4);
+            sp = sp1;
+#else
+#pragma unroll
+            for (int t = 0; t < T1; ++t)
+#pragma unroll
+                for (int v = 0; v < (t == T1 - 1 ? 8 : 16); v += 4)
+                    sp += pk(acc1[t][v], acc1[t][v + 1]) + pk(acc1[t][v + 2], acc1[t][v + 3]);
+#endif
+            const float s = sp[0] + sp[1];
+            const float mean = (s + __shfl_xor(s, 32)) * (1.f / H1);
+            nmean = pk(-mean, -mean);
+            f32x2 ssp = pk(0.f, 0.f);
+#pragma unroll
+            for (int t = 0; t < T1; ++t)
+#pragma unroll
+                for (int v = 0; v < (t == T1 - 1 ? 8 : 16); v += 2) {
+                    const f32x2 d = pk(acc1[t][v], acc1[t][v + 1]) + nmean;
+                    ssp = pk_fma(d, d, ssp);
+                }
+            const float ss = ssp[0] + ssp[1];
+            const float var = (ss + __shfl_xor(ss, 32)) * (1.f / H1) * (UNSCALE * UNSCALE);
+            const float rstd = rsqrtf(var + 1e-5f) * UNSCALE;
+            rstdp = pk(rstd, rstd);
+        }
+        constexpr int GROUPS = 2 * STEPS;
+        float4 gq[2], bq[2];
+        f32x2 ya, yb;
+        float y0, y1, y2, y3;
+        auto ln_read = [&](const int G) __attribute__((always_inline)) {
+            gq[G & 1] = lds4(pv1 + 8 * G);
+            bq[G & 1] = lds4(pv1 + H1P + 8 * G);
+        };
+        auto ln_chunk = [&](const int G, const int k) __attribute__((always_inline)) {
+            const int t = G >> 2, i = G & 3, st = G >> 1, e = 2 * (G & 1);
+            const float4 g = gq[G & 1], be = bq[G & 1];
+            if (k == 0) ya = pk_fma((pk(acc1[t][4 * i], acc1[t][4 * i + 1]) + nmean) * rstdp, pk(g.x, g.y), pk(be.x, be.y));
+            if (k == 1) yb = pk_fma((pk(acc1[t][4 * i + 2], acc1[t][4 * i + 3]) + nmean) * rstdp, pk(g.z, g.w), pk(be.z, be.w));
+            if (k == 2) {
+                y0 = fmaxf(ya[0], 0.f); y1 = fmaxf(ya[1], 0.f); y2 = fmaxf(yb[0], 0.f); y3 = fmaxf(yb[1], 0.f);
+                if (G + 1 < GROUPS) ln_read(G + 1);
+            }
+            if (k == 3) split2(y0, y1, hb[st][e], mb[st][e]);
+            if (k == 4) split2(y2, y3, hb[st][e + 1], mb[st][e + 1]);
+        };
+        ln_read(0);
+#pragma unroll
+        for (int G = 0; G < 4; ++G)
+#pragma unroll
+            for (int k = 0; k < 5; ++k) ln_chunk(G, k);
+
+        if (first) NSTAMP(3);
+        f32x16 acc2[T2];
+#pragma unroll
+        for (int u = 0; u < T2; ++u)
+#pragma unroll
+            for (int v = 0; v < 16; ++v) acc2[u][v] = 0.f;
+        asm volatile("s_waitcnt vmcnt(10)" ::: "memory");
+        __builtin_amdgcn_s_barrier();
+        uint4 c0h = lds_frag(LB, 0), c0m = lds_frag(LB, 1024), c1h = lds_frag(LB, 2048), c1m = lds_frag(LB, 3072), c2h = c0h, c2m = c0m;
+        SB;
+#if TT_SPLIT_SCHED == 1
+        f32x2 s2q = pk(0.f, 0.f);
+        float4 b2q[2][4];
+        auto pass_a_read = [&](const int w) __attribute__((always_inline)) {
+#pragma unroll
+            for (int i = 0; i < 4; ++i) b2q[w & 1][i] = lds4(pv2 + 32 * w + 8 * i);
+        };
+        auto pass_a = [&](const int w, const int i) __attribute__((always_inline)) {
+            const float4 b = b2q[w & 1][i];
+            const f32x2 xa = pk_fma(pk(acc2[w][4 * i], acc2[w][4 * i + 1]), pk(UNSCALE, UNSCALE), pk(b.x, b.y));
+            const f32x2 xb2 = pk_fma(pk(acc2[w][4 * i + 2], acc2[w][4 * i + 3]), pk(UNSCALE, UNSCALE), pk(b.z, b.w));
+            acc2[w][4 * i] = xa[0]; acc2[w][4 * i + 1] = xa[1]; acc2[w][4 * i + 2] = xb2[0]; acc2[w][4 * i + 3] = xb2[1];
+            s2q += xa + xb2;
+        };
+#endif
+        auto l2_step = [&](const int s) __attribute__((always_inline)) {
+            const uint4 vh = make_uint4(hb[s][0], hb[s][1], hb[s][2], hb[s][3]), vm = make_uint4(mb[s][0], mb[s][1], mb[s][2], mb[s][3]);
+            const int slot = (s % RING) * CHUNK_BYTES, nslot = ((s + 1) % RING) * CHUNK_BYTES;
+            const unsigned char *wsl_s = wsl_cur;
+            unsigned lds_s = ldsw_w2, lds1_s = ldsw_w1;
+            asm volatile("" : "+s"(wsl_s), "+s"(lds_s));
+            if (s >= TAIL0 && s < TAIL0 + 3) asm volatile("" : "+s"(lds1_s));
+#pragma unroll
+            for (int u = 0; u < T2; ++u) {
+#if TT_SPLIT_SCHED == 1
+                const bool pa = s == STEPS - 1 && u >= 2;
+#endif
+                if (u == T2 / 2 && s >= 1 && s + 1 < STEPS) {
+#if TT_SPLIT_SCHED == 1
+#define TT_WAIT_CASE(c) case c: asm volatile("s_waitcnt vmcnt(" #c ")" ::: "memory"); break;
+                    switch (L2S1[CRITIC].mid[s]) {
+                        TT_MID_CASES(TT_WAIT_CASE)
+                        default: asm volatile("s_waitcnt vmcnt(0)" ::: "memory"); break;
+                    }
+#undef TT_WAIT_CASE
+#else
+                    switch (L2S.mid[s]) {
+                        case 20: asm volatile("s_waitcnt vmcnt(20)" ::: "memory"); break;
+                        default: asm volatile("s_waitcnt vmcnt(18)" ::: "memory"); break;
+                    }
+#endif
+                    __builtin_amdgcn_s_barrier();
+                    SB;
+                }
+                const bool more = u + 2 < T2 || s + 1 < STEPS;
+                const int nx = u + 2 < T2 ? slot + (u + 2) * 2048 : nslot + (u + 2 - T2) * 2048;
+                acc2[u] = mfma_f16(c0h, vm, acc2[u]); SB;
+                if (more) c2h = lds_frag(LB, nx);
+                if (s + 2 < STEPS) ln_chunk(2 * (s + 2) + u / 5, u % 5);
+#if TT_SPLIT_SCHED == 1
+                if (pa) pass_a(u - 2, 0);
+#endif
+                SB;
+                acc2[u] = mfma_f16(c0m, vh, acc2[u]); SB;
+                if (more) c2m = lds_frag(LB, nx + 1024);
+#if TT_SPLIT_SCHED == 1
+                if (pa) pass_a(u - 2, 1);
+#endif
+                SB;
+                acc2[u] = mfma_f16(c0h, vh, acc2[u]); SB;
+#if TT_SPLIT_SCHED == 1
+                if (pa) { pass_a(u - 2, 2); pass_a(u - 2, 3); }
+                if (s == STEPS - 1 && u >= 1) pass_a_read(u - 1);
+#endif
+                {
+#if TT_SPLIT_SCHED == 1
+                    const int jl = L2S1[CRITIC].job[s][u];
+                    if (jl >= JOB_OBS && jl < JOB_RNG) load_next(tile, jl - JOB_OBS);
+                    if (!CRITIC && jl >= JOB_RNG) rng_piece(tile, jl - JOB_RNG);
+                    const int j = jl >= JOB_OBS ? JOB_NONE : jl;
+#else
+                    const int j = L2S.job[s][u];
+#endif
+                    const bool f1 = j >= JOB_FC1 && j < JOB_NEXT;
+                    const int st = j >= JOB_NEXT ? j - JOB_NEXT : j, i1 = j - JOB_FC1;
+                    if (j != JOB_NONE)
+                        dma_piece(wsl_s, f1 ? voff_w1 + i1 * 4096 : voff_w2 + st * CHUNK_BYTES + l2_piece(u) * 1024, f1 ? lds1_s : lds_s,
+                                  f1 ? i1 * 4096 : (st % RING) * CHUNK_BYTES + l2_piece(u) * 1024);
+                }
+                SB;
+                c0h = c1h; c0m = c1m; c1h = c2h; c1m = c2m;
+            }
+        };
+#pragma unroll
+        for (int s = 0; s < 2; ++s) l2_step(s);
+#if TT_SPLIT_SCHED == 1
+#define TT_L2_STEPS(a, b) _Pragma("unroll") for (int s = a; s < b; ++s) l2_step(s);
+        TT_L2_STEPS(2, 5) TT_L2_STEPS(5, 8) TT_L2_STEPS(8, 11) TT_L2_STEPS(11, 14) TT_L2_STEPS(14, 16) TT_L2_STEPS(16, 18)
+        TT_L2_STEPS(18, 20) TT_L2_STEPS(20, 22) TT_L2_STEPS(22, 24) TT_L2_STEPS(24, STEPS)
+#undef TT_L2_STEPS
+        static_assert(STEPS == 25, "the loops above cover steps 2..24");
+#else
+#pragma unroll
+        for (int s = 2; s < TAIL0; ++s) l2_step(s);
+#pragma unroll
+        for (int s = TAIL0; s < STEPS; ++s) l2_step(s);
+#endif
+#undef SB
+
+        if (first) NSTAMP(4);
+        const int next = tile + (int)gridDim.x;
+        const bool more_tiles = next < tile_end;
+#if TT_SPLIT_SCHED == 0
+        if (more_tiles) load_obs(next);
+#endif
+        f32x2 s2p = pk(0.f, 0.f);
+#if TT_SPLIT_SCHED == 1
+        pass_a_read(T2 - 1);
+#pragma unroll
+        for (int w = T2 - 2; w < T2; ++w)
+#pragma unroll
+            for (int i = 0; i < 4; ++i) pass_a(w, i);
+        s2p = s2q;
+#else
+        {
+            float4 bq[2][4];
+            auto ldb = [&](const int u, float4 (&b)[4]) {
+#pragma unroll
+                for (int i = 0; i < 4; ++i) b[i] = lds4(pv2 + 32 * u + 8 * i);
+            };
+            ldb(0, bq[0]);
+#pragma unroll
+            for (int u = 0; u < T2; ++u) {
+                if (u + 1 < T2) ldb(u + 1, bq[(u + 1) & 1]);
+                __builtin_amdgcn_sched_barrier(0);
+#pragma unroll
+                for (int i = 0; i < 4; ++i) {
+                    const float4 b = bq[u & 1][i];
+                    const f32x2 xa = pk_fma(pk(acc2[u][4 * i], acc2[u][4 * i + 1]), pk(UNSCALE, UNSCALE), pk(b.x, b.y));
+                    const f32x2 xb2 = pk_fma(pk(acc2[u][4 * i + 2], acc2[u][4 * i + 3]), pk(UNSCALE, UNSCALE), pk(b.z, b.w));
+                    acc2[u][4 * i] = xa[0]; acc2[u][4 * i + 1] = xa[1]; acc2[u][4 * i + 2] = xb2[0]; acc2[u][4 * i + 3] = xb2[1];
+                    s2p += xa + xb2;
+                }
+                __builtin_amdgcn_sched_barrier(0);
+            }
+        }
+#endif
+        const float s2 = s2p[0] + s2p[1];
+        const float mean2 = (s2 + __shfl_xor(s2, 32)) * (1.f / H2);
+        const f32x2 nmean2 = pk(-mean2, -mean2);
+        f32x2 ss2p = pk(0.f, 0.f);
+#pragma unroll
+        for (int u = 0; u < T2; ++u)
+#pragma unroll
+            for (int i = 0; i < 4; ++i) {
+                const bool real = 32 * u + 8 * i + 4 * h < H2;
+                const f32x2 keep = real ? pk(1.f, 1.f) : pk(0.f, 0.f);
+#pragma unroll
+                for (int j = 0; j < 4; j += 2) {
+                    const f32x2 d = pk(acc2[u][4 * i + j], acc2[u][4 * i + j + 1]) + nmean2;
+                    acc2[u][4 * i + j] = d[0]; acc2[u][4 * i + j + 1] = d[1];
+                    const f32x2 dk = (32 * u + 8 * i + 4 < H2) ? d : d * keep;
+                    ss2p = pk_fma(dk, dk, ss2p);
+                }
+            }
+        const float ss2 = ss2p[0] + ss2p[1];
+        const float rstd2 = rsqrtf((ss2 + __shfl_xor(ss2, 32)) * (1.f / H2) + 1e-5f);
+        const f32x2 rstd2p = pk(rstd2, rstd2);
+        const float av = (CRITIC && row < n) ? action[row] : 0.f;
+        f32x2 dotp = pk(0.f, 0.f);
+        {
+            constexpr int NV = CRITIC ? 5 : 3;
+            float4 vq[2][4][NV];
+            auto ldv = [&](const int u, float4 (&v)[4][NV]) {
+#pragma unroll
+                for (int i = 0; i < 4; ++i)
+#pragma unroll
+                    for (int q = 0; q < NV; ++q) v[i][q] = lds4(pv2 + (q + 1) * H2P + 32 * u + 8 * i);
+            };
+            ldv(0, vq[0]);
+#pragma unroll
+            for (int u = 0; u < T2; ++u) {
+                if (u + 1 < T2) ldv(u + 1, vq[(u + 1) & 1]);
+                __builtin_amdgcn_sched_barrier(0);
+#pragma unroll
+                for (int i = 0; i < 4; ++i) {
+                    const float4 g = vq[u & 1][i][0], be = vq[u & 1][i][1], w3 = vq[u & 1][i][2];
+                    f32x2 ya = pk_fma(pk(acc2[u][4 * i], acc2[u][4 * i + 1]) * rstd2p, pk(g.x, g.y), pk(be.x, be.y));
+                    f32x2 yb = pk_fma(pk(acc2[u][4 * i + 2], acc2[u][4 * i + 3]) * rstd2p, pk(g.z, g.w), pk(be.z, be.w));
+                    if (CRITIC) {
+                        const float4 wa = vq[u & 1][i][NV - 2], ba = vq[u & 1][i][NV - 1];
+                        ya += pk_fma(pk(av, av), pk(wa.x, wa.y), pk(ba.x, ba.y));
+                        yb += pk_fma(pk(av, av), pk(wa.z, wa.w), pk(ba.z, ba.w));
+                    }
+                    dotp = pk_fma(pk(fmaxf(ya[0], 0.f), fmaxf(ya[1], 0.f)), pk(w3.x, w3.y), dotp);
+                    dotp = pk_fma(pk(fmaxf(yb[0], 0.f), fmaxf(yb[1], 0.f)), pk(w3.z, w3.w), dotp);
+                }
+                __builtin_amdgcn_sched_barrier(0);
+            }
+        }
+        const float dot = dotp[0] + dotp[1];
+        const float v = dot + __shfl_xor(dot, 32) + lds4(pv1 - 4 * h + VEC_FLOATS).x;
+        if (h == 0 && row < n) {
+            if (with_noise) finish_row_noise(row, v, out, act, ou_next, araw);
+            else finish_row<CRITIC>(row, v, out, act);
+        }
+        if (first) NSTAMP(5);
+#ifdef TT_STAMPS
+        TSTAMP(round, 1);
+        if (threadIdx.x == 0 && blockIdx.x < 512 && round < 4) tt_log_add(g_log_tile, g_tile[blockIdx.x][round][0], g_tile[blockIdx.x][round][1]);
+        ++round;
+        if (more_tiles) TSTAMP(round, 0);
+#endif
+        if (!more_tiles) break;
+        tile = next;
+        first = false;
+    }
+    asm volatile("s_waitcnt vmcnt(0)" ::: "memory");
+}
diff --git a/ddpg-trucktrailer_amd/fused.py b/ddpg-trucktrailer_amd/fused.py
--- a/ddpg-trucktrailer_amd/fused.py
+++ b/ddpg-trucktrailer_amd/fused.py
@@ -131,9 +131,26 @@
     return act_scaled
 
 
+POLICY_KERNELS = ("k_mlp_split", "k_mlp_split_shadow")
+
+
+def policy_schedule():
+    return int(L.load().tt_mlp_split_schedule_set(-1))
+
+
+@contextlib.contextmanager
+def policy_schedule_as(schedule):
+    assert schedule in (0, 1)
+    prev = int(L.load().tt_mlp_split_schedule_set(int(schedule)))
+    try:
+        yield
+    finally:
+        L.load().tt_mlp_split_schedule_set(prev)
+
+
 def policy_kernel_info(n):
     waves = 4 * ((n + 127) // 128)
-    return {"kernel": "k_mlp_split (choose_action for N envs; split-f16; the image's pack launch, ~4 us per step, not included)",
+    return {"kernel": POLICY_KERNELS[policy_schedule()] + " (choose_action for N envs; split-f16; the image's pack launch, ~4 us per step, not included)",
             "mfma_flop": waves * (750 + 78) * 32768.0,
             "note": "f16 MFMA FLOP executed (three f16 products per f32 product block, both layers) over the dense f16/bf16 "
                     "peak; algorithmic_* = the network's useful f32 FLOP"}
diff --git a/include/ttenv.h b/include/ttenv.h
--- a/include/ttenv.h
+++ b/include/ttenv.h
@@ -158,6 +158,7 @@
     void *net, *target;
 } tt_fc2_images;
 uint64_t tt_mlp_split_ws_bytes(void);
+int tt_mlp_split_schedule_set(int schedule);
 int tt_mlp_split_pack(const tt_mlp_weights *w, int critic, void *ws, int64_t *bump, const tt_ring_cursor *cursor,
                       tt_stream_t stream);
 
```

Result: slower. 814.4 million (-2.3%).
